# mks0601/ExAvatar_RELEASE

Hardware: NVIDIA H100
Metric: avatar train-step frames/sec (fwd+bwd raster) (higher is better)
Workload: dtype f32

## Files before the change

exavatar_release_b200/_lib.py:

```python
from __future__ import annotations

import ctypes as C
import os

_PKG = os.path.dirname(os.path.abspath(__file__))
LIB_PATH = os.path.join(_PKG, "libb200raster.so")
LIB_PATH = os.environ.get("B2R_LIB", LIB_PATH)

ABI_VERSION = 3
B2R_OK = 0
B2R_FLAG_NO_TILE_CULL = 1
B2R_FLAG_DEBUG = 2
B2R_FLAG_CTX_CLEAN = 4

_fp = C.c_void_p


class B2RScene(C.Structure):
    _fields_ = [
        ("P", C.c_int32), ("width", C.c_int32), ("height", C.c_int32), ("sh_degree", C.c_int32),
        ("sh_coeffs", C.c_int32), ("flags", C.c_uint32),
        ("scale_modifier", C.c_float), ("tanfovx", C.c_float), ("tanfovy", C.c_float),
        ("bg", _fp), ("viewmatrix", _fp), ("projmatrix", _fp), ("campos", _fp),
        ("means3D", _fp), ("shs", _fp), ("colors_precomp", _fp), ("opacities", _fp),
        ("scales", _fp), ("rotations", _fp), ("cov3D_precomp", _fp),
        ("skin_xyz", _fp), ("skin_weights", _fp), ("skin_joint_mats", _fp), ("skin_trans", _fp),
        ("skin_cam_Rinv", _fp), ("skin_cam_t", _fp), ("skin_means_out", _fp), ("skin_J", C.c_int32),
        ("sh_rows", C.c_int32),
    ]


class B2RStatus(C.Structure):
    _fields_ = [
        ("num_dups", C.c_uint64), ("dup_capacity", C.c_uint64), ("overflow", C.c_uint32), ("num_visible", C.c_uint32),
        ("consumed_fwd", C.c_uint64), ("consumed_bwd", C.c_uint64), ("token", C.c_uint64), ("reserved", C.c_uint64 * 2),
    ]


class B2RWorkspace(C.Structure):
    _fields_ = [
        ("ctx", _fp), ("ctx_bytes", C.c_size_t), ("dup_ids", _fp), ("dup_capacity", C.c_uint64),
        ("scratch", _fp), ("scratch_bytes", C.c_size_t), ("status_mirror", _fp), ("status_token", C.c_uint64),
        ("checkpoints", _fp), ("checkpoint_bytes", C.c_size_t),
    ]


class B2RView(C.Structure):
    _fields_ = [
        ("id_begin", C.c_uint32), ("id_end", C.c_uint32), ("bg", _fp), ("final_T", _fp), ("n_contrib", _fp),
        ("checkpoints", _fp), ("checkpoint_bytes", C.c_size_t), ("skip_below", C.c_uint32), ("reserved", C.c_uint32),
    ]


class B2RSkin(C.Structure):
    _fields_ = [
        ("P", C.c_int32), ("J", C.c_int32), ("V", C.c_int32), ("reserved", C.c_int32),
        ("weights", _fp), ("rows", _fp), ("joint_mats", _fp), ("trans", _fp), ("cam_Rinv", _fp), ("cam_t", _fp),
        ("xyz", _fp * 2), ("posed", _fp * 2),
    ]


class B2RMeshRender(C.Structure):
    _fields_ = [
        ("V", C.c_int32), ("F", C.c_int32), ("Vt", C.c_int32), ("C", C.c_int32),
        ("tex_height", C.c_int32), ("tex_width", C.c_int32), ("height", C.c_int32), ("width", C.c_int32),
        ("mesh", _fp), ("faces", _fp), ("vertex_uv", _fp), ("face_uv", _fp), ("texture", _fp),
        ("cam_R", _fp), ("cam_t", _fp), ("focal", _fp), ("princpt", _fp), ("keys", _fp),
        ("vf_offsets", _fp), ("vf_entries", _fp),
    ]


class B2RForwardOutputs(C.Structure):
    _fields_ = [("color", _fp), ("depth", _fp), ("alpha", _fp), ("radii", _fp)]


class B2RBackwardArgs(C.Structure):
    _fields_ = [
        ("dL_dcolor", _fp), ("dL_ddepth", _fp), ("dL_dalpha", _fp),
        ("dL_dmeans3D", _fp), ("dL_dmeans2D", _fp), ("dL_dshs", _fp), ("dL_dcolors", _fp), ("dL_dopacities", _fp),
        ("dL_dscales", _fp), ("dL_drotations", _fp), ("dL_dcov3D", _fp),
        ("flags", C.c_uint32), ("first_row", C.c_uint32),
        ("densify_grad_accum", _fp), ("densify_count", _fp), ("densify_radius_max", _fp),
        ("dL_dskin_xyz", _fp), ("dL_dskin_G", _fp),
        ("dL_dposed", _fp),
        ("densify_rows", C.c_uint32), ("reserved", C.c_uint32),
    ]


CONSUMED_FWD_DIV = 8
CONSUMED_BWD_DIV = 4

B2R_BWD_ACCUMULATE = 1
B2R_BWD_SCRATCH_ZEROED = 2


def read_status(ctx_buf) -> dict:
    s = B2RStatus.from_buffer_copy(ctx_buf[: C.sizeof(B2RStatus)].cpu().numpy().tobytes())
    return {"num_dups": int(s.num_dups), "dup_capacity": int(s.dup_capacity), "overflow": int(s.overflow),
            "num_visible": int(s.num_visible), "consumed_fwd": int(s.consumed_fwd), "consumed_bwd": int(s.consumed_bwd),
            "consumed_fwd_div": float(CONSUMED_FWD_DIV), "consumed_bwd_div": float(CONSUMED_BWD_DIV)}


SYMBOLS = [
    ("b2r_abi_version", C.c_int, []),
    ("b2r_strerror", C.c_char_p, [C.c_int]),
    ("b2r_last_cuda_error", C.c_int, []),
    ("b2r_sizeof", C.c_size_t, [C.c_int]),
    ("b2r_ctx_bytes", C.c_size_t, [C.c_int32, C.c_int32, C.c_int32]),
    ("b2r_scratch_bytes", C.c_size_t, [C.c_int32, C.c_int32, C.c_int32, C.c_uint64]),
    ("b2r_backward_scratch_bytes", C.c_size_t, [C.c_int32]),
    ("b2r_checkpoint_bytes", C.c_size_t, [C.c_int32, C.c_int32, C.c_uint64]),
    ("b2r_forward_bin", C.c_int, [C.POINTER(B2RScene), C.POINTER(B2RWorkspace), _fp]),
    ("b2r_forward_composite", C.c_int, [C.POINTER(B2RScene), C.POINTER(B2RWorkspace), C.POINTER(B2RView),
                                        C.POINTER(B2RForwardOutputs), _fp]),
    ("b2r_backward_composite", C.c_int, [C.POINTER(B2RScene), C.POINTER(B2RWorkspace), C.POINTER(B2RView),
                                         C.POINTER(B2RBackwardArgs), _fp, C.c_size_t, _fp]),
    ("b2r_backward_project", C.c_int, [C.POINTER(B2RScene), C.POINTER(B2RWorkspace), C.POINTER(B2RBackwardArgs), _fp,
                                       C.c_size_t, _fp]),
    ("b2r_forward_project", C.c_int, [C.POINTER(B2RScene), C.POINTER(B2RWorkspace), _fp, _fp]),
    ("b2r_forward_render", C.c_int, [C.POINTER(B2RScene), C.POINTER(B2RWorkspace), C.POINTER(B2RForwardOutputs), _fp]),
    ("b2r_forward", C.c_int, [C.POINTER(B2RScene), C.POINTER(B2RWorkspace), C.POINTER(B2RForwardOutputs), _fp]),
    ("b2r_backward", C.c_int, [C.POINTER(B2RScene), C.POINTER(B2RWorkspace), C.POINTER(B2RBackwardArgs), _fp,
                               C.c_size_t, _fp]),
    ("b2r_mark_visible", C.c_int, [C.c_int32, _fp, _fp, _fp, _fp]),
    ("b2r_skin_forward", C.c_int, [C.POINTER(B2RSkin), _fp]),
    ("b2r_skin_backward", C.c_int, [C.POINTER(B2RSkin), C.POINTER(_fp), C.POINTER(_fp), _fp, _fp, _fp, C.c_size_t, _fp]),
    ("b2r_skin_scratch_bytes", C.c_size_t, [C.c_int32, C.c_int32]),
    ("b2r_l1ssim_scratch_bytes", C.c_size_t, [C.c_int32, C.c_int32]),
    ("b2r_l1ssim_forward", C.c_int, [C.c_int32, C.c_int32, _fp, _fp, _fp, _fp, C.c_int32, _fp, _fp, C.c_size_t, _fp]),
    ("b2r_l1ssim_backward", C.c_int, [C.c_int32, C.c_int32, _fp, _fp, _fp, _fp, C.c_int32, _fp, _fp, _fp, C.c_size_t,
                                      _fp]),
    ("b2r_nearest_scratch_bytes", C.c_size_t, [C.c_int32, C.c_int32]),
    ("b2r_nearest_rows", C.c_int, [C.c_int32, _fp, C.c_int32, _fp, _fp, _fp, _fp, C.c_size_t, _fp]),
    ("b2r_vertex_normals", C.c_int, [C.c_int32, _fp, _fp, _fp, _fp, _fp, _fp, _fp]),
    ("b2r_mesh_render_scratch_bytes", C.c_size_t, [C.c_int32]),
    ("b2r_mesh_render_forward", C.c_int, [C.POINTER(B2RMeshRender), _fp, _fp, _fp, C.c_size_t, _fp]),
    ("b2r_mesh_render_backward", C.c_int, [C.POINTER(B2RMeshRender), _fp, _fp, _fp, _fp, C.c_size_t, _fp]),
    ("b2r_profile_enable", None, [C.c_int]),
    ("b2r_profile_read", C.c_int, [C.POINTER(C.c_double), C.POINTER(C.c_uint64), C.c_int]),
    ("b2r_launch_count", C.c_uint64, []),
    ("b2r_kernel_name", C.c_char_p, [C.c_int]),
    ("b2r_ctx_geom", _fp, [C.POINTER(B2RWorkspace), C.c_int32, C.c_int32, C.c_int32]),
    ("b2r_ctx_aux", _fp, [C.POINTER(B2RWorkspace), C.c_int32, C.c_int32, C.c_int32]),
    ("b2r_ctx_ranges", _fp, [C.POINTER(B2RWorkspace), C.c_int32, C.c_int32, C.c_int32]),
    ("b2r_ctx_final_T", _fp, [C.POINTER(B2RWorkspace), C.c_int32, C.c_int32, C.c_int32]),
    ("b2r_ctx_n_contrib", _fp, [C.POINTER(B2RWorkspace), C.c_int32, C.c_int32, C.c_int32]),
]

_lib = None


def load():
    global _lib
    if _lib is not None:
        return _lib
    if not os.path.exists(LIB_PATH):
        raise RuntimeError(
            f"b200raster: {LIB_PATH} not found. Build it with `python -m exavatar_release_b200.build_ext` "
            "(nvcc, sm_90a). There is no CPU fallback.")
    lib = C.CDLL(LIB_PATH)
    for name, restype, argtypes in SYMBOLS:
        fn = getattr(lib, name)
        fn.restype = restype
        fn.argtypes = argtypes
    if lib.b2r_abi_version() != ABI_VERSION:
        raise RuntimeError("b200raster: ABI version mismatch between the Python binding and libb200raster.so")
    for idx, cls in ((0, B2RScene), (1, B2RStatus), (2, B2RWorkspace), (3, B2RForwardOutputs), (4, B2RBackwardArgs),
                     (5, B2RView), (6, B2RSkin), (8, B2RMeshRender)):
        if lib.b2r_sizeof(idx) != C.sizeof(cls):
            raise RuntimeError(f"b200raster: struct layout drift for {cls.__name__}: "
                               f"{lib.b2r_sizeof(idx)} (C) vs {C.sizeof(cls)} (ctypes)")
    _lib = lib
    return lib


def check(rc: int, what: str):
    if rc != B2R_OK:
        lib = load()
        msg = lib.b2r_strerror(rc).decode()
        raise RuntimeError(f"b200raster: {what} failed: {msg} (code {rc}, cudaError {lib.b2r_last_cuda_error()})")
```

exavatar_release_b200/csrc/api.cu:

```cuda
#include "common.cuh"

using namespace b2r;

namespace {

int validate_scene(const B2RScene* sc) {
  if (!sc) return B2R_E_INVALID;
  if (sc->P < 0 || sc->width <= 0 || sc->height <= 0) return B2R_E_INVALID;
  if (sc->P >= (1 << 29)) return B2R_E_INVALID;
  if (sc->width > 65535 * TILE || sc->height > 32767 * TILE) return B2R_E_INVALID;
  if (!(sc->tanfovx > 0.f) || !(sc->tanfovy > 0.f)) return B2R_E_INVALID;
  if (!sc->bg || !sc->viewmatrix || !sc->projmatrix || !sc->campos) return B2R_E_INVALID;
  if (sc->sh_rows < 0 || sc->sh_rows > sc->P) return B2R_E_INVALID;
  if (sc->P > 0) {
    if (!sc->opacities) return B2R_E_INVALID;
    if (sc->skin_xyz) {
      if (!sc->skin_weights || !sc->skin_joint_mats || !sc->skin_trans) return B2R_E_INVALID;
      if (sc->skin_J <= 0 || sc->skin_J > 64) return B2R_E_INVALID;
      if (sc->skin_cam_Rinv && !sc->skin_cam_t) return B2R_E_INVALID;
    } else if (!sc->means3D) {
      return B2R_E_INVALID;
    }
    if (sc->sh_rows > 0) {
      if (!sc->shs || !sc->colors_precomp) return B2R_E_INVALID;
    } else if ((sc->shs != nullptr) == (sc->colors_precomp != nullptr)) {
      return B2R_E_INVALID;
    }
    const bool sr = sc->scales != nullptr && sc->rotations != nullptr;
    if (sr == (sc->cov3D_precomp != nullptr)) return B2R_E_INVALID;
    if ((sc->scales != nullptr) != (sc->rotations != nullptr)) return B2R_E_INVALID;
    if (sc->shs) {
      if (sc->sh_degree < 0 || sc->sh_degree > 3) return B2R_E_INVALID;
      if (sc->sh_coeffs < (sc->sh_degree + 1) * (sc->sh_degree + 1)) return B2R_E_INVALID;
      if (sc->sh_coeffs > 16) return B2R_E_INVALID;
    }
  }
  return B2R_OK;
}

int validate_ws(const B2RScene* sc, const B2RWorkspace* ws, bool need_scratch) {
  if (!ws || !ws->ctx) return B2R_E_INVALID;
  if (ws->ctx_bytes < b2r_ctx_bytes(sc->P, sc->width, sc->height)) return B2R_E_WORKSPACE;
  if (ws->dup_capacity > 0xfffffff0ull) return B2R_E_INVALID;
  if (need_scratch) {
    if (!ws->scratch) return B2R_E_INVALID;
    if (ws->scratch_bytes < b2r_scratch_bytes(sc->P, sc->width, sc->height, ws->dup_capacity)) return B2R_E_WORKSPACE;
  }
  if (ws->dup_capacity > 0 && !ws->dup_ids) return B2R_E_INVALID;
  if (ws->checkpoints && ws->checkpoint_bytes < b2r_checkpoint_bytes(sc->width, sc->height, ws->dup_capacity)) return B2R_E_WORKSPACE;
  return B2R_OK;
}

bool missing_dshs(const B2RScene* sc, const B2RBackwardArgs* a) {
  if (!sc->shs || a->dL_dshs || sc->P == 0) return false;
  return sc->sh_rows == 0 || (int64_t)a->first_row < (int64_t)sc->sh_rows;
}

int validate_skin(const B2RSkin* s) {
  if (!s) return B2R_E_INVALID;
  if (s->P < 0 || s->V <= 0) return B2R_E_INVALID;
  if (s->J <= 0 || s->J > 64) return B2R_E_INVALID;
  if (s->cam_Rinv && !s->cam_t) return B2R_E_INVALID;
  if (s->posed[1] && !s->xyz[1]) return B2R_E_INVALID;
  if (s->P > 0) {
    if (!s->weights || !s->joint_mats || !s->trans || !s->xyz[0]) return B2R_E_INVALID;
    if (!s->rows && s->V < s->P) return B2R_E_INVALID;
  }
  return B2R_OK;
}

bool valid_l1ssim_size(int32_t width, int32_t height) {
  return width > 0 && height > 0 && height <= 65535 * 16 && (int64_t)width * height <= (int64_t)1 << 31;
}

int validate_mesh_render(const B2RMeshRender* m) {
  if (!m) return B2R_E_INVALID;
  if (m->V < 0 || m->F < 0 || m->Vt < 0 || m->C < 1 || m->C > 4) return B2R_E_INVALID;
  if (m->width <= 0 || m->height <= 0 || (int64_t)m->width * m->height >= ((int64_t)1 << 31)) return B2R_E_INVALID;
  if (m->F >= (1 << 29) || m->V >= (1 << 29)) return B2R_E_INVALID;
  if (!m->cam_R || !m->cam_t || !m->focal || !m->princpt) return B2R_E_INVALID;
  if (m->F > 0) {
    if (m->V < 1 || m->Vt < 1 || m->tex_height < 1 || m->tex_width < 1) return B2R_E_INVALID;
    if ((int64_t)m->C * m->tex_height * m->tex_width >= ((int64_t)1 << 31)) return B2R_E_INVALID;
    if (!m->mesh || !m->faces || !m->vertex_uv || !m->face_uv || !m->texture) return B2R_E_INVALID;
  }
  return B2R_OK;
}

}

extern "C" {

int b2r_abi_version(void) { return B2R_ABI_VERSION; }

const char* b2r_strerror(int code) {
  switch (code) {
    case B2R_OK: return "ok";
    case B2R_E_INVALID: return "invalid argument";
    case B2R_E_WORKSPACE: return "workspace buffer too small";
    case B2R_E_CUDA: return "CUDA launch failed";
    case B2R_E_DUP_OVERFLOW: return "duplicate capacity exceeded";
    default: return "unknown error";
  }
}

int b2r_last_cuda_error(void) { return g_last_cuda_error; }

size_t b2r_sizeof(int which) {
  switch (which) {
    case 0: return sizeof(B2RScene);
    case 1: return sizeof(B2RStatus);
    case 2: return sizeof(B2RWorkspace);
    case 3: return sizeof(B2RForwardOutputs);
    case 4: return sizeof(B2RBackwardArgs);
    case 5: return sizeof(B2RView);
    case 6: return sizeof(B2RSkin);
    case 8: return sizeof(B2RMeshRender);
    default: return 0;
  }
}

size_t b2r_ctx_bytes(int32_t P, int32_t width, int32_t height) { return ctx_layout(P, width, height).total; }

size_t b2r_scratch_bytes(int32_t P, int32_t width, int32_t height, uint64_t dup_capacity) {
  return scratch_layout(P, width, height, dup_capacity).total;
}

size_t b2r_backward_scratch_bytes(int32_t P) { return align_up((size_t)(P > 0 ? P : 1) * 12 * sizeof(float)); }

size_t b2r_checkpoint_bytes(int32_t width, int32_t height, uint64_t dup_capacity) {
  const CtxLayout L = ctx_layout(0, width, height);
  const uint32_t ms = max_segments(L.tiles, dup_capacity);
  return seg_table_bytes(ms) + (size_t)ms * CK_REC_BYTES;
}

int b2r_forward_project(const B2RScene* scene, const B2RWorkspace* ws, int32_t* radii, void* stream) {
  int rc = validate_scene(scene);
  if (rc) return rc;
  rc = validate_ws(scene, ws, false);
  if (rc) return rc;
  if (scene->P > 0 && !radii) return B2R_E_INVALID;
  const Ctx cx = resolve(ws, scene->P, scene->width, scene->height);
  return launch_project(*scene, cx, radii, (cudaStream_t)stream);
}

static int forward_render(const B2RScene* scene, const B2RWorkspace* ws, const B2RForwardOutputs* out, bool rescan,
                          void* stream) {
  int rc = validate_scene(scene);
  if (rc) return rc;
  rc = validate_ws(scene, ws, true);
  if (rc) return rc;
  if (!out || !out->color || !out->depth || !out->alpha) return B2R_E_INVALID;
  const Ctx cx = resolve(ws, scene->P, scene->width, scene->height);
  rc = launch_binning(*scene, cx, rescan, (cudaStream_t)stream);
  if (rc) return rc;
  return launch_composite_fwd(*scene, cx, *out, (cudaStream_t)stream);
}

static int apply_view(Ctx& cx, const B2RScene* scene, const B2RWorkspace* ws, const B2RView* v) {
  if (!v) return B2R_OK;
  if (v->id_end < v->id_begin || (int64_t)v->id_end > (int64_t)scene->P) return B2R_E_INVALID;
  if ((v->final_T != nullptr) != (v->n_contrib != nullptr)) return B2R_E_INVALID;
  cx.id_begin = v->id_begin;
  cx.id_span = v->id_end - v->id_begin;
  cx.bg = v->bg;
  cx.skip_below = v->skip_below;
  if (v->final_T) { cx.final_T = v->final_T; cx.n_contrib = v->n_contrib; }
  if (v->checkpoints && cx.ckpt) {
    const size_t need = seg_table_bytes(cx.max_segs) + (size_t)cx.max_segs * CK_REC_BYTES;
    if (v->checkpoint_bytes < need) return B2R_E_WORKSPACE;
    cx.ckpt = (float*)((char*)v->checkpoints + seg_table_bytes(cx.max_segs));
  }
  (void)ws;
  return B2R_OK;
}

int b2r_forward_bin(const B2RScene* scene, const B2RWorkspace* ws, void* stream) {
  int rc = validate_scene(scene);
  if (rc) return rc;
  rc = validate_ws(scene, ws, true);
  if (rc) return rc;
  const Ctx cx = resolve(ws, scene->P, scene->width, scene->height);
  return launch_binning(*scene, cx, false, (cudaStream_t)stream);
}

int b2r_forward_composite(const B2RScene* scene, const B2RWorkspace* ws, const B2RView* view,
                          const B2RForwardOutputs* out, void* stream) {
  int rc = validate_scene(scene);
  if (rc) return rc;
  rc = validate_ws(scene, ws, false);
  if (rc) return rc;
  if (!out || !out->color || !out->depth || !out->alpha) return B2R_E_INVALID;
  Ctx cx = resolve(ws, scene->P, scene->width, scene->height);
  rc = apply_view(cx, scene, ws, view);
  if (rc) return rc;
  return launch_composite_fwd(*scene, cx, *out, (cudaStream_t)stream);
}

int b2r_forward_render(const B2RScene* scene, const B2RWorkspace* ws, const B2RForwardOutputs* out, void* stream) {
  return forward_render(scene, ws, out, true, stream);
}

int b2r_forward(const B2RScene* scene, const B2RWorkspace* ws, const B2RForwardOutputs* out, void* stream) {
  if (!out) return B2R_E_INVALID;
  int rc = b2r_forward_project(scene, ws, out->radii, stream);
  if (rc) return rc;
  return forward_render(scene, ws, out, false, stream);
}

int b2r_backward(const B2RScene* scene, const B2RWorkspace* ws, const B2RBackwardArgs* args, void* bwd_scratch,
                 size_t bwd_scratch_bytes, void* stream) {
  int rc = validate_scene(scene);
  if (rc) return rc;
  rc = validate_ws(scene, ws, false);
  if (rc) return rc;
  if (!args || !args->dL_dcolor || !bwd_scratch) return B2R_E_INVALID;
  if (bwd_scratch_bytes < b2r_backward_scratch_bytes(scene->P)) return B2R_E_WORKSPACE;
  if (missing_dshs(scene, args)) return B2R_E_INVALID;
  if ((int64_t)args->first_row > (int64_t)scene->P) return B2R_E_INVALID;
  if (args->dL_dposed && !scene->skin_xyz) return B2R_E_INVALID;
  const Ctx cx = resolve(ws, scene->P, scene->width, scene->height);
  float* gacc = (float*)bwd_scratch;
  rc = launch_composite_bwd(*scene, cx, *args, gacc, (cudaStream_t)stream);
  if (rc) return rc;
  return launch_project_bwd(*scene, cx, *args, gacc, (cudaStream_t)stream);
}

int b2r_backward_composite(const B2RScene* scene, const B2RWorkspace* ws, const B2RView* view, const B2RBackwardArgs* args,
                           void* bwd_scratch, size_t bwd_scratch_bytes, void* stream) {
  int rc = validate_scene(scene);
  if (rc) return rc;
  rc = validate_ws(scene, ws, false);
  if (rc) return rc;
  if (!args || !args->dL_dcolor || !bwd_scratch) return B2R_E_INVALID;
  if (bwd_scratch_bytes < b2r_backward_scratch_bytes(scene->P)) return B2R_E_WORKSPACE;
  if ((int64_t)args->first_row > (int64_t)scene->P) return B2R_E_INVALID;
  Ctx cx = resolve(ws, scene->P, scene->width, scene->height);
  rc = apply_view(cx, scene, ws, view);
  if (rc) return rc;
  return launch_composite_bwd(*scene, cx, *args, (float*)bwd_scratch, (cudaStream_t)stream);
}

int b2r_backward_project(const B2RScene* scene, const B2RWorkspace* ws, const B2RBackwardArgs* args, void* bwd_scratch,
                         size_t bwd_scratch_bytes, void* stream) {
  int rc = validate_scene(scene);
  if (rc) return rc;
  rc = validate_ws(scene, ws, false);
  if (rc) return rc;
  if (!args || !bwd_scratch) return B2R_E_INVALID;
  if (bwd_scratch_bytes < b2r_backward_scratch_bytes(scene->P)) return B2R_E_WORKSPACE;
  if (missing_dshs(scene, args)) return B2R_E_INVALID;
  if ((int64_t)args->first_row > (int64_t)scene->P) return B2R_E_INVALID;
  if (args->dL_dposed && !scene->skin_xyz) return B2R_E_INVALID;
  const Ctx cx = resolve(ws, scene->P, scene->width, scene->height);
  return launch_project_bwd(*scene, cx, *args, (const float*)bwd_scratch, (cudaStream_t)stream);
}

size_t b2r_skin_scratch_bytes(int32_t P, int32_t J) { return skin_scratch_bytes(P, J); }

int b2r_skin_forward(const B2RSkin* skin, void* stream) {
  const int rc = validate_skin(skin);
  if (rc) return rc;
  if (skin->P > 0 && !skin->posed[0]) return B2R_E_INVALID;
  return launch_skin_forward(*skin, (cudaStream_t)stream);
}

int b2r_skin_backward(const B2RSkin* skin, const float* const dL_dposed[2], float* const dL_dxyz[2], float* dL_djoint,
                      float* dL_dtrans, void* scratch, size_t scratch_bytes, void* stream) {
  const int rc = validate_skin(skin);
  if (rc) return rc;
  if (dL_dposed && dL_dposed[1] && !skin->xyz[1]) return B2R_E_INVALID;
  if ((dL_djoint || dL_dtrans) && skin->P > 0) {
    if (!scratch) return B2R_E_INVALID;
    if (scratch_bytes < skin_scratch_bytes(skin->P, skin->J)) return B2R_E_WORKSPACE;
  }
  return launch_skin_backward(*skin, dL_dposed, dL_dxyz, dL_djoint, dL_dtrans, scratch, (cudaStream_t)stream);
}

size_t b2r_l1ssim_scratch_bytes(int32_t width, int32_t height) { return l1ssim_scratch_bytes(width, height); }

int b2r_l1ssim_forward(int32_t width, int32_t height, const float* img, const float* target, const float* mask,
                       const float* bbox, int32_t with_ssim, float* out, void* scratch, size_t scratch_bytes,
                       void* stream) {
  if (!valid_l1ssim_size(width, height) || !img || !target || !out || !scratch) return B2R_E_INVALID;
  if (scratch_bytes < l1ssim_scratch_bytes(width, height)) return B2R_E_WORKSPACE;
  return launch_l1ssim_forward(width, height, img, target, mask, bbox, with_ssim != 0, out, scratch,
                               (cudaStream_t)stream);
}

int b2r_l1ssim_backward(int32_t width, int32_t height, const float* img, const float* target, const float* mask,
                        const float* bbox, int32_t with_ssim, const float* dL_dout, float* dL_dimg, const void* scratch,
                        size_t scratch_bytes, void* stream) {
  if (!valid_l1ssim_size(width, height) || !img || !target || !dL_dout || !dL_dimg) return B2R_E_INVALID;
  if (with_ssim) {
    if (!scratch) return B2R_E_INVALID;
    if (scratch_bytes < l1ssim_scratch_bytes(width, height)) return B2R_E_WORKSPACE;
  }
  return launch_l1ssim_backward(width, height, img, target, mask, bbox, with_ssim != 0, dL_dout, dL_dimg, scratch,
                                (cudaStream_t)stream);
}

size_t b2r_nearest_scratch_bytes(int32_t P, int32_t V) {
  (void)P;
  return nearest_scratch_bytes(V);
}

int b2r_nearest_rows(int32_t P, const float* queries, int32_t V, const float* targets, const uint8_t* self_map,
                     int32_t* rows, void* scratch, size_t scratch_bytes, void* stream) {
  if (P < 0 || V < 0 || V >= (1 << 29)) return B2R_E_INVALID;
  if (P == 0) return B2R_OK;
  if (V < 1 || !queries || !targets || !rows || !scratch) return B2R_E_INVALID;
  if (scratch_bytes < nearest_scratch_bytes(V)) return B2R_E_WORKSPACE;
  return launch_nearest_rows(P, queries, V, targets, self_map, rows, scratch, (cudaStream_t)stream);
}

int b2r_vertex_normals(int32_t P, const float* xyz, const int32_t* faces, const int32_t* vf_offsets,
                       const int32_t* vf_entries, const uint8_t* flip, float* normals, void* stream) {
  if (P < 0) return B2R_E_INVALID;
  if (P == 0) return B2R_OK;
  if (!xyz || !faces || !vf_offsets || !vf_entries || !normals) return B2R_E_INVALID;
  return launch_vertex_normals(P, xyz, faces, vf_offsets, vf_entries, flip, normals, (cudaStream_t)stream);
}

size_t b2r_mesh_render_scratch_bytes(int32_t F) { return mesh_render_scratch_bytes(F); }

int b2r_mesh_render_forward(const B2RMeshRender* mr, float* image, int32_t* pix_to_face, void* scratch,
                            size_t scratch_bytes, void* stream) {
  const int rc = validate_mesh_render(mr);
  if (rc) return rc;
  if (!mr->keys || !image || !pix_to_face || !scratch) return B2R_E_INVALID;
  if (scratch_bytes < mesh_render_scratch_bytes(mr->F)) return B2R_E_WORKSPACE;
  return launch_mesh_render_forward(*mr, image, pix_to_face, scratch, (cudaStream_t)stream);
}

int b2r_mesh_render_backward(const B2RMeshRender* mr, const int32_t* pix_to_face, const float* dL_dimage,
                             float* dL_dmesh, void* scratch, size_t scratch_bytes, void* stream) {
  const int rc = validate_mesh_render(mr);
  if (rc) return rc;
  if (!pix_to_face || !dL_dimage || !scratch) return B2R_E_INVALID;
  if (mr->V > 0 && (!dL_dmesh || !mr->vf_offsets || !mr->vf_entries)) return B2R_E_INVALID;
  if (scratch_bytes < mesh_render_scratch_bytes(mr->F)) return B2R_E_WORKSPACE;
  return launch_mesh_render_backward(*mr, pix_to_face, dL_dimage, dL_dmesh, scratch, (cudaStream_t)stream);
}

int b2r_mark_visible(int32_t P, const float* means3D, const float* viewmatrix, uint8_t* present, void* stream) {
  if (P < 0 || (P > 0 && (!means3D || !present)) || !viewmatrix) return B2R_E_INVALID;
  return launch_mark_visible(P, means3D, viewmatrix, present, (cudaStream_t)stream);
}

const float* b2r_ctx_geom(const B2RWorkspace* ws, int32_t P, int32_t width, int32_t height) {
  return (const float*)((const char*)ws->ctx + ctx_layout(P, width, height).geom);
}
const int32_t* b2r_ctx_aux(const B2RWorkspace* ws, int32_t P, int32_t width, int32_t height) {
  return (const int32_t*)((const char*)ws->ctx + ctx_layout(P, width, height).aux);
}
const uint32_t* b2r_ctx_ranges(const B2RWorkspace* ws, int32_t P, int32_t width, int32_t height) {
  return (const uint32_t*)((const char*)ws->ctx + ctx_layout(P, width, height).ranges);
}
const float* b2r_ctx_final_T(const B2RWorkspace* ws, int32_t P, int32_t width, int32_t height) {
  return (const float*)((const char*)ws->ctx + ctx_layout(P, width, height).final_T);
}
const uint32_t* b2r_ctx_n_contrib(const B2RWorkspace* ws, int32_t P, int32_t width, int32_t height) {
  return (const uint32_t*)((const char*)ws->ctx + ctx_layout(P, width, height).n_contrib);
}

}
```

exavatar_release_b200/csrc/binning.cu:

```cuda
#include <cstdlib>

#include "common.cuh"

namespace b2r {

__global__ void __launch_bounds__(256) scatter_kernel(const B2RScene sc, const Ctx cx) {
  const int i = blockIdx.x * blockDim.x + threadIdx.x;
  int4 aux = make_int4(0, 0, 0, 0);
  float4 g0 = make_float4(0.f, 0.f, 0.f, 0.f), g1 = g0;
  uint32_t depth_bits = 0u;
  if (i < sc.P) {
    aux = cx.aux[i];
    if (aux.z > 0) {
      const int area = ((aux.y & 0xffff) - (aux.x & 0xffff)) * ((aux.y >> 16) - (aux.x >> 16));
      depth_bits = __float_as_uint(cx.geom[i].g1.z);
      if (area > 32) {
        g0 = reinterpret_cast<const float4*>(cx.geom + i)[0];
        g1 = reinterpret_cast<const float4*>(cx.geom + i)[1];
      }
    }
  }
  const uint64_t cap = cx.dup_capacity;
  const int gx = cx.gx;
  uint32_t* cursor = cx.tile_cursor;
  uint2* keys = cx.keys;
  constexpr uint32_t NONE = 0xffffffffu;
  uint32_t pend_pos = NONE, pend_depth = 0, pend_id = 0;
  warp_replay_kept_tiles(aux.z > 0, aux.x & 0xffff, aux.x >> 16, aux.y & 0xffff, aux.y >> 16, (uint32_t)aux.w, g0.x, g0.y,
                         g0.z, g0.w, g1.x, g1.w, depth_bits, (uint32_t)i, (sc.flags & B2R_FLAG_NO_TILE_CULL) != 0, sc.width,
                         sc.height, gx, cursor, [&](uint32_t p, int, uint32_t d, uint32_t id) {
                           if (pend_pos < cap) keys[pend_pos] = make_uint2(pend_depth, pend_id);
                           pend_pos = p; pend_depth = d; pend_id = id;
                         });
  if (pend_pos < cap) keys[pend_pos] = make_uint2(pend_depth, pend_id);
}

__global__ void __launch_bounds__(256) scatter_agg_kernel(const B2RScene sc, const Ctx cx) {
  extern __shared__ uint32_t s_mem[];
  uint32_t* s_cnt = s_mem;
  uint32_t* s_base = s_mem + cx.tiles;
  for (int t = threadIdx.x; t < cx.tiles; t += blockDim.x) s_cnt[t] = 0u;
  __syncthreads();
  const int i = blockIdx.x * blockDim.x + threadIdx.x;
  int4 aux = make_int4(0, 0, 0, 0);
  float4 g0 = make_float4(0.f, 0.f, 0.f, 0.f), g1 = g0;
  uint32_t depth_bits = 0u;
  if (i < sc.P) {
    aux = cx.aux[i];
    if (aux.z > 0) {
      const int area = ((aux.y & 0xffff) - (aux.x & 0xffff)) * ((aux.y >> 16) - (aux.x >> 16));
      depth_bits = __float_as_uint(cx.geom[i].g1.z);
      if (area > 32) {
        g0 = reinterpret_cast<const float4*>(cx.geom + i)[0];
        g1 = reinterpret_cast<const float4*>(cx.geom + i)[1];
      }
    }
  }
  const int gx = cx.gx;
  const bool no_cull = (sc.flags & B2R_FLAG_NO_TILE_CULL) != 0;
  const int x0 = aux.x & 0xffff, y0 = aux.x >> 16, x1 = aux.y & 0xffff, y1 = aux.y >> 16;
  const uint32_t kept = (uint32_t)aux.w;
  warp_replay_kept_tiles(aux.z > 0, x0, y0, x1, y1, kept, g0.x, g0.y, g0.z, g0.w, g1.x, g1.w, 0u, 0u, no_cull, sc.width,
                         sc.height, gx, s_cnt, [](uint32_t, int, uint32_t, uint32_t) {});
  __syncthreads();
  for (int t = threadIdx.x; t < cx.tiles; t += blockDim.x) {
    const uint32_t c = s_cnt[t];
    if (c) {
      s_base[t] = atomicAdd(cx.tile_cursor + t, c);
      s_cnt[t] = 0u;
    }
  }
  __syncthreads();
  const uint64_t cap = cx.dup_capacity;
  uint2* keys = cx.keys;
  warp_replay_kept_tiles(aux.z > 0, x0, y0, x1, y1, kept, g0.x, g0.y, g0.z, g0.w, g1.x, g1.w, depth_bits, (uint32_t)i,
                         no_cull, sc.width, sc.height, gx, s_cnt, [&](uint32_t rank, int t, uint32_t d, uint32_t id) {
                           const uint32_t pos = s_base[t] + rank;
                           if (pos < cap) keys[pos] = make_uint2(d, id);
                         });
}


__device__ __forceinline__ unsigned match_digit(const uint32_t d, const bool valid) {
  unsigned peers = __ballot_sync(0xffffffffu, valid);
#pragma unroll
  for (int bit = 0; bit < 8; bit++) {
    const bool on = (d >> bit) & 1u;
    const unsigned b = __ballot_sync(0xffffffffu, on);
    peers &= on ? b : ~b;
  }
  return valid ? peers : 0u;
}

template <int CAP, int THREADS>
struct RadixSmem {
  static constexpr int W = THREADS / 32;
  static constexpr size_t bytes = (size_t)CAP * 12 + (size_t)W * 256 * 2 + 64;
};

template <int CAP, int THREADS, bool PAIRS = false>
__device__ __forceinline__ void radix_sort_tile(const uint2* src, uint32_t* dst, const int n, unsigned char* smem_raw,
                                                uint32_t* maxid) {
  constexpr int W = THREADS / 32;
  constexpr int ROWS = CAP / (W * 32);
  static_assert(CAP % (W * 32) == 0, "a warp's share must be whole rows");
  uint32_t* keyA = reinterpret_cast<uint32_t*>(smem_raw);
  uint32_t* keyB = keyA + CAP;
  uint16_t* idxA = reinterpret_cast<uint16_t*>(keyB + CAP);
  uint16_t* idxB = idxA + CAP;
  uint16_t* hist = idxB + CAP;
  uint32_t* misc = reinterpret_cast<uint32_t*>(hist + W * 256);
  const int tid = threadIdx.x, lane = tid & 31, warp = tid >> 5;

  if (tid == 0) { misc[0] = 0u; misc[1] = 0xffffffffu; }
  __syncthreads();
  uint32_t vor = 0u, vand = 0xffffffffu;
  for (int i = tid; i < n; i += THREADS) {
    const uint32_t k = src[i].x;
    keyA[i] = k;
    idxA[i] = (uint16_t)i;
    vor |= k;
    vand &= k;
  }
  vor = __reduce_or_sync(0xffffffffu, vor);
  vand = __reduce_and_sync(0xffffffffu, vand);
  if (lane == 0) { atomicOr(&misc[0], vor); atomicAnd(&misc[1], vand); }
  __syncthreads();
  const uint32_t differ = misc[0] ^ misc[1];

  const int chunk = (((n + W - 1) / W) + 31) & ~31;
  const int c_begin = min(warp * chunk, n), c_end = min(c_begin + chunk, n);
  uint32_t* kin = keyA; uint32_t* kout = keyB;
  uint16_t* iin = idxA; uint16_t* iout = idxB;
  for (int pass = 0; pass < 4; pass++) {
    const int shift = 8 * pass;
    if (((differ >> shift) & 0xffu) == 0u) continue;
    for (int i = tid; i < W * 256; i += THREADS) hist[i] = 0;
    __syncthreads();
    uint16_t* myhist = hist + warp * 256;
    unsigned row_peers[ROWS];
#pragma unroll
    for (int r = 0; r < ROWS; r++) {
      const int base = c_begin + 32 * r;
      row_peers[r] = 0u;
      if (base < c_end) {
        const int i = base + lane;
        const bool valid = i < c_end;
        const uint32_t d = valid ? ((kin[i] >> shift) & 0xffu) : (256u + lane);
        const unsigned peers = match_digit(d, valid);
        row_peers[r] = peers;
        if (valid && (peers & ((1u << lane) - 1u)) == 0u) myhist[d] = (uint16_t)(myhist[d] + __popc(peers));
        __syncwarp();
      }
    }
    __syncthreads();
    constexpr int DPT = THREADS >= 256 ? 1 : 256 / THREADS;
    constexpr int SCAN_THREADS = 256 / DPT;
    uint32_t tot[DPT];
    uint32_t total = 0;
    if (tid < SCAN_THREADS) {
#pragma unroll
      for (int r = 0; r < DPT; r++) {
        const int d = tid * DPT + r;
        uint32_t run = 0;
        for (int w = 0; w < W; w++) {
          const uint32_t t = hist[w * 256 + d];
          hist[w * 256 + d] = (uint16_t)run;
          run += t;
        }
        tot[r] = run;
        total += run;
      }
    }
    uint32_t incl = total;
#pragma unroll
    for (int o = 1; o < 32; o <<= 1) {
      const uint32_t v = __shfl_up_sync(0xffffffffu, incl, o);
      if (lane >= o) incl += v;
    }
    if (tid < SCAN_THREADS && lane == 31) misc[2 + warp] = incl;
    __syncthreads();
    if (tid < SCAN_THREADS) {
      uint32_t base = incl - total;
      for (int w = 0; w < warp; w++) base += misc[2 + w];
#pragma unroll
      for (int r = 0; r < DPT; r++) {
        const int d = tid * DPT + r;
        for (int w = 0; w < W; w++) hist[w * 256 + d] = (uint16_t)(hist[w * 256 + d] + base);
        base += tot[r];
      }
    }
    __syncthreads();
#pragma unroll
    for (int r = 0; r < ROWS; r++) {
      const int base = c_begin + 32 * r;
      if (base < c_end) {
        const int i = base + lane;
        const bool valid = i < c_end;
        const uint32_t k = valid ? kin[i] : 0u;
        const uint32_t d = (k >> shift) & 0xffu;
        const unsigned peers = row_peers[r];
        const unsigned below = peers & ((1u << lane) - 1u);
        uint32_t start = 0;
        if (valid && below == 0u) {
          start = myhist[d];
          myhist[d] = (uint16_t)(start + __popc(peers));
        }
        start = __shfl_sync(0xffffffffu, start, valid ? __ffs(peers) - 1 : lane);
        if (valid) {
          const uint32_t o = start + __popc(below);
          kout[o] = k;
          iout[o] = iin[i];
        }
        __syncwarp();
      }
    }
    __syncthreads();
    { uint32_t* t = kin; kin = kout; kout = t; }
    { uint16_t* t = iin; iin = iout; iout = t; }
  }
  uint32_t* ids = kout;
  uint32_t vmax = 0u;
  for (int i = tid; i < n; i += THREADS) {
    const uint32_t id = src[iin[i]].y;
    ids[i] = id;
    vmax = max(vmax, id);
  }
  vmax = __reduce_max_sync(0xffffffffu, vmax);
  if (lane == 0 && vmax) atomicMax(maxid, vmax);
  __syncthreads();
  for (;;) {
    int changed = 0;
#pragma unroll
    for (int phase = 0; phase < 2; phase++) {
      for (int i = 2 * tid + phase; i + 1 < n; i += 2 * THREADS) {
        if (kin[i] == kin[i + 1]) {
          const uint32_t a = ids[i], b = ids[i + 1];
          if (a > b) { ids[i] = b; ids[i + 1] = a; changed = 1; }
        }
      }
      __syncthreads();
    }
    if (!__syncthreads_or(changed)) break;
  }
  if (PAIRS) {
    uint2* out = const_cast<uint2*>(src);
    for (int i = tid; i < n; i += THREADS) out[i] = make_uint2(kin[i], ids[i]);
  } else {
    for (int i = tid; i < n; i += THREADS) dst[i] = ids[i];
  }
  __syncthreads();
}

constexpr int WSORT_CAP = 1 << SORT_CTA_SHIFT;
constexpr size_t WSORT_BYTES = (size_t)WSORT_CAP * 12 + 256 * 2;

__device__ __forceinline__ void warp_sort_tile(const uint2* __restrict__ src, uint32_t* __restrict__ dst, const int n,
                                               unsigned char* smem_warp, uint32_t* __restrict__ maxid) {
  const int lane = threadIdx.x & 31;
  const unsigned below_mask = (1u << lane) - 1u;
  if (n <= 0) return;
  if (n <= 32) {
    const uint2 kv = lane < n ? src[lane] : make_uint2(0xffffffffu, 0xffffffffu);
    const uint32_t m = __reduce_max_sync(0xffffffffu, lane < n ? kv.y : 0u);
    if (lane == 0) *maxid = m;
    const unsigned long long me = ((unsigned long long)kv.x << 32) | kv.y;
    int rank = 0;
    for (int j = 0; j < n; j++) {
      const unsigned long long o = __shfl_sync(0xffffffffu, me, j);
      rank += (o < me) ? 1 : 0;
    }
    if (lane < n) dst[rank] = kv.y;
    return;
  }
  uint32_t* keyA = reinterpret_cast<uint32_t*>(smem_warp);
  uint32_t* keyB = keyA + WSORT_CAP;
  uint16_t* idxA = reinterpret_cast<uint16_t*>(keyB + WSORT_CAP);
  uint16_t* idxB = idxA + WSORT_CAP;
  uint16_t* hist = idxB + WSORT_CAP;
  uint32_t vor = 0u, vand = 0xffffffffu;
  for (int i = lane; i < n; i += 32) {
    const uint32_t k = src[i].x;
    keyA[i] = k;
    idxA[i] = (uint16_t)i;
    vor |= k;
    vand &= k;
  }
  const uint32_t differ = __reduce_or_sync(0xffffffffu, vor) ^ __reduce_and_sync(0xffffffffu, vand);
  __syncwarp();
  uint32_t* kin = keyA; uint32_t* kout = keyB;
  uint16_t* iin = idxA; uint16_t* iout = idxB;
  for (int pass = 0; pass < 4; pass++) {
    const int shift = 8 * pass;
    if (((differ >> shift) & 0xffu) == 0u) continue;
    reinterpret_cast<uint4*>(hist)[lane] = make_uint4(0u, 0u, 0u, 0u);
    __syncwarp();
    constexpr int CACHED = 8;
    unsigned row_peers[CACHED];
#pragma unroll
    for (int r = 0; r < CACHED; r++) {
      const int base = 32 * r;
      row_peers[r] = 0u;
      if (base < n) {
        const int i = base + lane;
        const bool valid = i < n;
        const uint32_t d = valid ? ((kin[i] >> shift) & 0xffu) : (256u + lane);
        const unsigned peers = match_digit(d, valid);
        row_peers[r] = peers;
        if (valid && (peers & below_mask) == 0u) hist[d] = (uint16_t)(hist[d] + __popc(peers));
        __syncwarp();
      }
    }
    for (int base = 32 * CACHED; base < n; base += 32) {
      const int i = base + lane;
      const bool valid = i < n;
      const uint32_t d = valid ? ((kin[i] >> shift) & 0xffu) : (256u + lane);
      const unsigned peers = match_digit(d, valid);
      if (valid && (peers & below_mask) == 0u) hist[d] = (uint16_t)(hist[d] + __popc(peers));
      __syncwarp();
    }
    uint32_t c[8], total = 0;
#pragma unroll
    for (int r = 0; r < 8; r++) { c[r] = hist[8 * lane + r]; total += c[r]; }
    uint32_t incl = total;
#pragma unroll
    for (int o = 1; o < 32; o <<= 1) {
      const uint32_t v = __shfl_up_sync(0xffffffffu, incl, o);
      if (lane >= o) incl += v;
    }
    uint32_t run = incl - total;
#pragma unroll
    for (int r = 0; r < 8; r++) { hist[8 * lane + r] = (uint16_t)run; run += c[r]; }
    __syncwarp();
    auto place_row = [&](const int base, const bool cached, const unsigned cached_peers) {
        const int i = base + lane;
        const bool valid = i < n;
        const uint32_t k = valid ? kin[i] : 0u;
        const uint32_t d = valid ? ((k >> shift) & 0xffu) : (256u + lane);
        const unsigned peers = cached ? cached_peers : match_digit(d, valid);
        const unsigned below = peers & below_mask;
        uint32_t start = 0;
        if (valid && below == 0u) {
          start = hist[d];
          hist[d] = (uint16_t)(start + __popc(peers));
        }
        start = __shfl_sync(0xffffffffu, start, valid ? __ffs(peers) - 1 : lane);
        if (valid) {
          const uint32_t o = start + __popc(below);
          kout[o] = k;
          iout[o] = iin[i];
        }
        __syncwarp();
    };
#pragma unroll
    for (int r = 0; r < CACHED; r++)
      if (32 * r < n) place_row(32 * r, true, row_peers[r]);
    for (int base = 32 * CACHED; base < n; base += 32) place_row(base, false, 0u);
    { uint32_t* t = kin; kin = kout; kout = t; }
    { uint16_t* t = iin; iin = iout; iout = t; }
  }
  uint32_t* ids = kout;
  uint32_t vmax = 0u;
  for (int i = lane; i < n; i += 32) {
    const uint32_t id = src[iin[i]].y;
    ids[i] = id;
    vmax = max(vmax, id);
  }
  vmax = __reduce_max_sync(0xffffffffu, vmax);
  if (lane == 0) *maxid = vmax;
  __syncwarp();
  for (;;) {
    bool changed = false;
#pragma unroll
    for (int phase = 0; phase < 2; phase++) {
      for (int i = 2 * lane + phase; i + 1 < n; i += 64) {
        if (kin[i] == kin[i + 1]) {
          const uint32_t a = ids[i], b = ids[i + 1];
          if (a > b) { ids[i] = b; ids[i + 1] = a; changed = true; }
        }
      }
      __syncwarp();
    }
    if (!__any_sync(0xffffffffu, changed)) break;
  }
  for (int i = lane; i < n; i += 32) dst[i] = ids[i];
  __syncwarp();
}

template <int CAP, int THREADS>
__global__ void __launch_bounds__(THREADS) sort_mixed_kernel(const Ctx cx) {
  extern __shared__ __align__(16) unsigned char smem_raw[];
  B2R_TRACE_BEGIN();
  const unsigned long long cls = cx.status->reserved[0];
  const int n_large = (int)(cls & 0xffffffffull), n_ge512 = (int)(cls >> 32);
  const int n_chunks = (int)cx.status->reserved[1];
  const int n_cta = n_ge512 - n_large;
  const int n_warp_items = (cx.tiles - n_ge512 + (THREADS / 32) - 1) / (THREADS / 32);
  const int items = n_chunks + n_cta + n_warp_items;
  int last_n = 0;
  for (int b = blockIdx.x; b < items; b += gridDim.x) {
    if (b < n_chunks) {
      int lo = 0, hi = n_large - 1;
      while (lo < hi) {
        const int mid = (lo + hi + 1) >> 1;
        if ((int)cx.chunk_start[mid] <= b) lo = mid; else hi = mid - 1;
      }
      const uint32_t tile = cx.tile_order[lo];
      const uint2 r = cx.ranges[tile];
      const int off = (b - (int)cx.chunk_start[lo]) * SORT_CHUNK;
      const int len = min(SORT_CHUNK, (int)(r.y - r.x) - off);
      if (len > 1) radix_sort_tile<CAP, THREADS, true>(cx.keys + r.x + off, nullptr, len, smem_raw, cx.tile_maxid + tile);
      else if (len == 1 && threadIdx.x == 0) atomicMax(cx.tile_maxid + tile, cx.keys[r.x + off].y);
      last_n = len;
    } else if (b < n_chunks + n_cta) {
      const uint32_t tile = cx.tile_order[n_large + (b - n_chunks)];
      const uint2 r = cx.ranges[tile];
      const int n = (int)(r.y - r.x);
      const uint2* src = cx.keys + r.x;
      uint32_t* dst = cx.dup_ids + r.x;
      if (n > 32) {
        radix_sort_tile<CAP, THREADS>(src, dst, n, smem_raw, cx.tile_maxid + tile);
      } else {
        if (threadIdx.x < 32) warp_sort_tile(src, dst, n, smem_raw, cx.tile_maxid + tile);
        __syncthreads();
      }
      last_n = n;
    } else {
      const int warp = threadIdx.x >> 5;
      const int t = n_ge512 + (b - n_chunks - n_cta) * (THREADS / 32) + warp;
      if (t < cx.tiles) {
        const uint32_t tile = cx.tile_order[t];
        const uint2 r = cx.ranges[tile];
        last_n = -(int)(r.y - r.x);
        warp_sort_tile(cx.keys + r.x, cx.dup_ids + r.x, (int)(r.y - r.x), smem_raw + (size_t)warp * WSORT_BYTES,
                       cx.tile_maxid + tile);
      }
    }
  }
  B2R_TRACE_END(last_n);
}

constexpr int MERGE_TABLE = 1024;
__global__ void __launch_bounds__(256) merge_chunks_kernel(const Ctx cx) {
  const int n_large = (int)(cx.status->reserved[0] & 0xffffffffull);
  const int n_chunks = (int)cx.status->reserved[1];
  if ((int)blockIdx.x >= n_chunks) return;
  __shared__ uint2 other[SORT_CHUNK];
  __shared__ uint32_t table[MERGE_TABLE];
  const int tid = threadIdx.x;
  const int n_tab = min(n_large, MERGE_TABLE);
  for (int i = tid; i < n_tab; i += 256) table[i] = cx.chunk_start[i];
  __syncthreads();
  constexpr int PER = SORT_CHUNK / 256;
  for (int b = blockIdx.x; b < n_chunks; b += gridDim.x) {
    int lo = 0, hi = n_large - 1;
    while (lo < hi) {
      const int mid = (lo + hi + 1) >> 1;
      const int cs = mid < n_tab ? (int)table[mid] : (int)cx.chunk_start[mid];
      if (cs <= b) lo = mid; else hi = mid - 1;
    }
    const uint2 r = cx.ranges[cx.tile_order[lo]];
    const int n = (int)(r.y - r.x);
    const int c = b - (int)(lo < n_tab ? table[lo] : cx.chunk_start[lo]);
    const uint2* pairs = cx.keys + r.x;
    const int chunks = (n + SORT_CHUNK - 1) / SORT_CHUNK;
    const int len = min(SORT_CHUNK, n - c * SORT_CHUNK);
    unsigned long long key[PER];
    uint32_t id[PER];
    int rank[PER];
#pragma unroll
    for (int j = 0; j < PER; j++) {
      const int i = j * 256 + tid;
      const uint2 me = i < len ? pairs[c * SORT_CHUNK + i] : make_uint2(0u, 0u);
      key[j] = ((unsigned long long)me.x << 32) | me.y;
      id[j] = me.y;
      rank[j] = i;
    }
    for (int c2 = 0; c2 < chunks; c2++) {
      if (c2 == c) continue;
      const uint2* q = pairs + c2 * SORT_CHUNK;
      const int len2 = min(SORT_CHUNK, n - c2 * SORT_CHUNK);
      __syncthreads();
#pragma unroll
      for (int j = 0; j < PER; j++) {
        const int i = j * 256 + tid;
        if (i < len2) other[i] = q[i];
      }
      __syncthreads();
      int l[PER];
#pragma unroll
      for (int j = 0; j < PER; j++) l[j] = 0;
#pragma unroll
      for (int step = SORT_CHUNK / 2; step >= 1; step >>= 1) {
#pragma unroll
        for (int j = 0; j < PER; j++) {
          const int probe = l[j] + step;
          if (probe <= len2) {
            const uint2 v = other[probe - 1];
            if ((((unsigned long long)v.x << 32) | v.y) < key[j]) l[j] = probe;
          }
        }
      }
      if (len2 == SORT_CHUNK) {
#pragma unroll
        for (int j = 0; j < PER; j++) {
          if (l[j] == SORT_CHUNK - 1) {
            const uint2 v = other[SORT_CHUNK - 1];
            if ((((unsigned long long)v.x << 32) | v.y) < key[j]) l[j] = SORT_CHUNK;
          }
        }
      }
#pragma unroll
      for (int j = 0; j < PER; j++) rank[j] += l[j];
    }
#pragma unroll
    for (int j = 0; j < PER; j++)
      if (j * 256 + tid < len) cx.dup_ids[r.x + rank[j]] = id[j];
  }
}

constexpr int SORT_SMALL = SORT_CHUNK;

int launch_binning(const B2RScene& sc, const Ctx& cx, bool rescan, cudaStream_t st) {
  if (rescan) {
    Ctx quiet = cx;
    quiet.status_mirror = nullptr;
    launch_tile_scan(quiet, st);
  }
  if (sc.P > 0) {
    ProfScope p(K_SCATTER, st);
    const size_t smem = (size_t)cx.tiles * 8;
    if (cx.tiles <= 2048) {
      cudaFuncSetAttribute(scatter_agg_kernel, cudaFuncAttributeMaxDynamicSharedMemorySize, 96 * 1024);
      launch_k(scatter_agg_kernel, (sc.P + 255) / 256, 256, smem, st, true, sc, cx);
    } else {
      launch_k(scatter_kernel, (sc.P + 255) / 256, 256, 0, st, true, sc, cx);
    }
  }
  const int sms = device_sm_count();
  constexpr int ST = 256;
  constexpr size_t cta_bytes = RadixSmem<SORT_SMALL, ST>::bytes, warp_bytes = (ST / 32) * WSORT_BYTES;
  constexpr size_t small_bytes = cta_bytes > warp_bytes ? cta_bytes : warp_bytes;
  cudaFuncSetAttribute(sort_mixed_kernel<SORT_SMALL, ST>, cudaFuncAttributeMaxDynamicSharedMemorySize, (int)small_bytes);
  {
    ProfScope p(K_SORT_SMALL, st);
    launch_k(sort_mixed_kernel<SORT_SMALL, ST>, cx.tiles, ST, small_bytes, st, true, cx);
  }
  {
    ProfScope p(K_SORT_LARGE, st);
    launch_k(merge_chunks_kernel, 2 * sms, 256, 0, st, true, cx);
  }
  return check_launch();
}

}

#ifdef B2R_CTA_TRACE
extern "C" int b2r_debug_trace_sort(unsigned long long* buf) {
  return (int)cudaMemcpyToSymbol(b2r::g_cta_trace, &buf, sizeof(buf));
}
#endif
```

exavatar_release_b200/csrc/common.cuh:

```cuda
#pragma once
#include <cuda_runtime.h>
#include <stdint.h>

#include "../../include/b200raster.h"

namespace b2r {

constexpr int TILE = 16;
constexpr int TILE_PIX = TILE * TILE;
constexpr float K_NEAR = 0.2f;
constexpr float K_DILATE = 0.3f;
constexpr float K_ALPHA_MAX = 0.99f;
constexpr float K_ALPHA_MIN = 1.0f / 255.0f;
constexpr float K_T_MIN = 0.0001f;
constexpr float K_FRUSTUM = 1.3f;
constexpr float K_EPS_W = 0.0000001f;
constexpr float K_EIG_FLOOR = 0.1f;
constexpr float LOG2E = 1.4426950408889634f;
constexpr float INV_LOG2E = 0.6931471805599453f;
constexpr float CULL_MARGIN2 = 0.02f;

#ifndef SORT_CTA_SHIFT
#define SORT_CTA_SHIFT 9
#endif
constexpr int SORT_CHUNK = 2048;
#ifndef SEG_SHIFT
#define SEG_SHIFT 9
#endif
constexpr int SEG = 1 << SEG_SHIFT;
constexpr int CK_PLANE0 = TILE_PIX * 4;
constexpr int CK_REC_FLOATS = TILE_PIX * 4 + TILE_PIX * 2;
constexpr size_t CK_REC_BYTES = (size_t)CK_REC_FLOATS * 4;
enum { CLS_N_LARGE = 0,
       CLS_N_GE512 = 1,
       CLS_N_MULTI = 2,
       CLS_N_CHUNKS = 3,
       CLS_TOTAL_SEGS = 4,
       CLS_N_GE1024 = 5,
       CLS_VIS_ACC = 6,
       CLS_SCAN_FINAL = 7,
       CLS_COUNT = 8 };
constexpr size_t ALIGN = 256;
__host__ __device__ inline size_t align_up(size_t v) { return (v + ALIGN - 1) / ALIGN * ALIGN; }

struct Geom {
  float4 g0;
  float4 g1;
  float4 g2;
};
static_assert(sizeof(Geom) == 48, "Geom must be 48 bytes");

struct CtxLayout {
  size_t status, geom, aux, ranges, tile_count, tile_cursor, tile_order, chunk_start, seg_start, classes, tile_maxid,
      final_T, n_contrib, total;
  int gx, gy, tiles;
};
__host__ __device__ inline CtxLayout ctx_layout(int P, int W, int H) {
  CtxLayout L;
  L.gx = (W + TILE - 1) / TILE;
  L.gy = (H + TILE - 1) / TILE;
  L.tiles = L.gx * L.gy;
  size_t Pn = P > 0 ? (size_t)P : 1, N = (size_t)W * H;
  size_t o = 0;
  L.status = o; o += align_up(sizeof(B2RStatus));
  L.geom = o; o += align_up(Pn * sizeof(Geom));
  L.aux = o; o += align_up(Pn * 16);
  L.ranges = o; o += align_up((size_t)L.tiles * 8);
  L.tile_count = o; o += align_up((size_t)L.tiles * 4);
  L.tile_cursor = o; o += align_up((size_t)L.tiles * 4);
  L.tile_order = o; o += align_up((size_t)L.tiles * 4);
  L.chunk_start = o; o += align_up((size_t)L.tiles * 4);
  L.seg_start = o; o += align_up((size_t)L.tiles * 4);
  L.classes = o; o += align_up((size_t)CLS_COUNT * 4);
  L.tile_maxid = o; o += align_up((size_t)L.tiles * 4);
  L.final_T = o; o += align_up(N * 4);
  L.n_contrib = o; o += align_up(N * 4);
  L.total = o;
  return L;
}

struct ScratchLayout {
  size_t keys, total;
};
__host__ __device__ inline ScratchLayout scratch_layout(int P, int W, int H, uint64_t cap) {
  (void)P; (void)W; (void)H;
  ScratchLayout S;
  size_t o = 0;
  S.keys = o; o += align_up((size_t)(cap > 0 ? cap : 1) * 8);
  S.total = o;
  return S;
}

struct Ctx {
  B2RStatus* status;
  Geom* geom;
  int4* aux;
  uint2* ranges;
  float* final_T;
  uint32_t* n_contrib;
  uint32_t* dup_ids;
  uint64_t dup_capacity;
  uint32_t* tile_count;
  uint32_t* tile_cursor;
  uint32_t* tile_order;
  uint32_t* chunk_start;
  uint2* keys;
  uint64_t* status_mirror;
  uint64_t status_token;
  int gx, gy, tiles;
  uint32_t* seg_start;
  uint32_t* classes;
  uint2* seg_table;
  float* ckpt;
  uint32_t max_segs;
  uint32_t id_begin, id_span;
  const float* bg;
  uint32_t* tile_maxid;
  uint32_t skip_below;
};

__host__ __device__ inline uint32_t max_segments(int tiles, uint64_t cap) { return (uint32_t)(cap / SEG) + (uint32_t)tiles; }
__host__ __device__ inline size_t seg_table_bytes(uint32_t max_segs) { return align_up((size_t)max_segs * 8); }

inline Ctx resolve(const B2RWorkspace* ws, int P, int W, int H) {
  CtxLayout L = ctx_layout(P, W, H);
  ScratchLayout S = scratch_layout(P, W, H, ws->dup_capacity);
  char* c = (char*)ws->ctx;
  char* s = (char*)ws->scratch;
  Ctx x;
  x.status = (B2RStatus*)(c + L.status);
  x.geom = (Geom*)(c + L.geom);
  x.aux = (int4*)(c + L.aux);
  x.ranges = (uint2*)(c + L.ranges);
  x.final_T = (float*)(c + L.final_T);
  x.n_contrib = (uint32_t*)(c + L.n_contrib);
  x.dup_ids = ws->dup_ids;
  x.dup_capacity = ws->dup_capacity;
  x.tile_count = (uint32_t*)(c + L.tile_count);
  x.tile_cursor = (uint32_t*)(c + L.tile_cursor);
  x.tile_order = (uint32_t*)(c + L.tile_order);
  x.chunk_start = (uint32_t*)(c + L.chunk_start);
  x.keys = s ? (uint2*)(s + S.keys) : nullptr;
  x.status_mirror = ws->status_mirror;
  x.status_token = ws->status_token;
  x.gx = L.gx; x.gy = L.gy; x.tiles = L.tiles;
  x.seg_start = (uint32_t*)(c + L.seg_start);
  x.classes = (uint32_t*)(c + L.classes);
  x.seg_table = nullptr; x.ckpt = nullptr; x.max_segs = 0;
  if (ws->checkpoints) {
    const uint32_t ms = max_segments(L.tiles, ws->dup_capacity);
    if (ws->checkpoint_bytes >= seg_table_bytes(ms) + (size_t)ms * CK_REC_BYTES) {
      x.seg_table = (uint2*)ws->checkpoints;
      x.ckpt = (float*)((char*)ws->checkpoints + seg_table_bytes(ms));
      x.max_segs = ms;
    }
  }
  x.id_begin = 0; x.id_span = 0xffffffffu;
  x.bg = nullptr;
  x.tile_maxid = (uint32_t*)(c + L.tile_maxid);
  x.skip_below = 0;
  return x;
}

__device__ __forceinline__ float region_max_p2(float sx, float sy, float A2, float B2, float C2, float x0, float y0,
                                               float x1, float y1) {
  const float lx = sx - x1, hx = sx - x0;
  const float ly = sy - y1, hy = sy - y0;
  const bool in_x = (lx <= 0.f) && (hx >= 0.f);
  const bool in_y = (ly <= 0.f) && (hy >= 0.f);
  if (in_x && in_y) return 0.f;
  float best = -INFINITY;
  if (!in_x) {
    const float ex = lx > 0.f ? lx : hx;
    float dy = __fdividef(-B2 * ex, 2.f * C2);
    dy = fminf(fmaxf(dy, ly), hy);
    best = fmaxf(best, A2 * ex * ex + B2 * ex * dy + C2 * dy * dy);
  }
  if (!in_y) {
    const float ey = ly > 0.f ? ly : hy;
    float dx = __fdividef(-B2 * ey, 2.f * A2);
    dx = fminf(fmaxf(dx, lx), hx);
    best = fmaxf(best, A2 * dx * dx + B2 * dx * ey + C2 * ey * ey);
  }
  return best;
}

struct RowCull {
  float sx, sy, A2, B2, nD4, fA4t, dy_ext, dys, inv2A;
  int mode;
};
__device__ __forceinline__ RowCull row_cull_setup(float sx, float sy, float A2, float B2, float C2, float thr2, bool no_cull) {
  RowCull rc;
  rc.sx = sx; rc.sy = sy; rc.A2 = A2; rc.B2 = B2;
  rc.mode = (no_cull || thr2 == -INFINITY) ? 1 : 0;
  const float D = B2 * B2 - 4.f * A2 * C2;
  const float k = __fdividef(4.f * thr2, -D);
  rc.dy_ext = sqrtf(A2 * k);
  const float dx_top = sqrtf(C2 * k);
  rc.dys = __fdividef(-B2, 2.f * C2) * dx_top;
  rc.nD4 = D;
  rc.fA4t = 4.f * A2 * thr2;
  rc.inv2A = __fdividef(1.f, 2.f * A2);
  if (rc.mode == 0 && !(rc.dy_ext >= 0.f)) rc.mode = 2;
  return rc;
}
constexpr float ROW_PAD = 0.01f;
__device__ __forceinline__ void row_kept_columns(const RowCull& rc, int ty, int x0, int x1, int W, int H, int& tlo, int& thi) {
  tlo = x0; thi = x1 - 1;
  if (rc.mode == 1) return;
  if (rc.mode == 2) { thi = tlo - 1; return; }
  const float y0 = (float)(ty * TILE), y1 = fminf(y0 + (float)(TILE - 1), (float)(H - 1));
  const float lo = fmaxf(rc.sy - y1, -rc.dy_ext), hi = fminf(rc.sy - y0, rc.dy_ext);
  if (!(lo <= hi)) { thi = tlo - 1; return; }
  const float dyr = fminf(fmaxf(rc.dys, lo), hi), dyl = fminf(fmaxf(-rc.dys, lo), hi);
  const float disc_r = fmaxf(rc.nD4 * dyr * dyr + rc.fA4t, 0.f), disc_l = fmaxf(rc.nD4 * dyl * dyl + rc.fA4t, 0.f);
  const float dx_hi = (-rc.B2 * dyr - sqrtf(disc_r)) * rc.inv2A;
  const float dx_lo = (-rc.B2 * dyl + sqrtf(disc_l)) * rc.inv2A;
  const float xl = rc.sx - dx_hi - ROW_PAD, xr = rc.sx - dx_lo + ROW_PAD;
  if (!(xl <= (float)(W - 1))) { thi = tlo - 1; return; }
  tlo = max(x0, (int)ceilf((xl - (float)(TILE - 1)) * (1.f / TILE)));
  thi = min(x1 - 1, (int)floorf(xr * (1.f / TILE)));
}

__device__ __forceinline__ int rect_row(int t, float inv_w) { return (int)(((float)t + 0.5f) * inv_w); }

constexpr int KEPT_SMALL = 4;
#ifndef WALK_ROW_COST_N
#define WALK_ROW_COST_N 40
#endif
constexpr unsigned WALK_ROW_COST = WALK_ROW_COST_N, WALK_TILE_COST = 10u, WALK_BCAST_COST = 30u;

__device__ __forceinline__ uint32_t bit_run(int pos, int cnt) { return (cnt >= 32 ? 0xffffffffu : ((1u << cnt) - 1u)) << pos; }

__device__ __forceinline__ uint32_t warp_count_kept_tiles(bool active, int x0, int y0, int x1, int y1, float px, float py,
                                                          float A2, float B2, float C2, float thr2, bool no_cull, int W,
                                                          int H, int gx, uint32_t* table) {
  const int lane = threadIdx.x & 31;
  const int w = x1 - x0, h = y1 - y0;
  const int area = active ? w * h : 0;
  uint32_t kept = 0u;
  const bool big = area > KEPT_SMALL;
  const unsigned own_cost = area ? (unsigned)h * WALK_ROW_COST + (unsigned)area * WALK_TILE_COST : 0u;
  const unsigned coop_cost = big ? WALK_BCAST_COST + (unsigned)((h + 31) >> 5) * (WALK_ROW_COST + (unsigned)w * WALK_TILE_COST) : 0u;
  const unsigned max_own = __reduce_max_sync(0xffffffffu, own_cost);
  const unsigned sum_coop = __reduce_add_sync(0xffffffffu, coop_cost);
  const bool all_private = max_own <= sum_coop + 64u;
  if (area > 0 && (all_private || !big)) {
    const RowCull rc = row_cull_setup(px, py, A2, B2, C2, thr2, no_cull);
    for (int ty = y0; ty < y1; ty++) {
      int tlo, thi;
      row_kept_columns(rc, ty, x0, x1, W, H, tlo, thi);
      if (tlo <= thi) {
        if (area <= 32) kept |= bit_run((ty - y0) * w + (tlo - x0), thi - tlo + 1);
        uint32_t* row = table + ty * gx;
        for (int tx = tlo; tx <= thi; tx++) atomicAdd(row + tx, 1u);
      }
    }
  }
  unsigned mask = all_private ? 0u : __ballot_sync(0xffffffffu, big);
  while (mask) {
    const int src = __ffs(mask) - 1;
    mask &= mask - 1;
    const int bx0 = __shfl_sync(0xffffffffu, x0, src), by0 = __shfl_sync(0xffffffffu, y0, src);
    const int bx1 = __shfl_sync(0xffffffffu, x1, src), by1 = __shfl_sync(0xffffffffu, y1, src);
    const float spx = __shfl_sync(0xffffffffu, px, src), spy = __shfl_sync(0xffffffffu, py, src);
    const float sA = __shfl_sync(0xffffffffu, A2, src), sB = __shfl_sync(0xffffffffu, B2, src);
    const float sC = __shfl_sync(0xffffffffu, C2, src), sT = __shfl_sync(0xffffffffu, thr2, src);
    const RowCull rc = row_cull_setup(spx, spy, sA, sB, sC, sT, no_cull);
    const int bw = bx1 - bx0;
    const bool small = bw * (by1 - by0) <= 32;
    uint32_t bits = 0u;
    for (int ty = by0 + lane; ty < by1; ty += 32) {
      int tlo, thi;
      row_kept_columns(rc, ty, bx0, bx1, W, H, tlo, thi);
      if (tlo <= thi) {
        if (small) bits |= bit_run((ty - by0) * bw + (tlo - bx0), thi - tlo + 1);
        uint32_t* row = table + ty * gx;
        for (int tx = tlo; tx <= thi; tx++) atomicAdd(row + tx, 1u);
      }
    }
    bits = __reduce_or_sync(0xffffffffu, bits);
    if (lane == src) kept = bits;
  }
  return kept;
}

template <typename F>
__device__ __forceinline__ void warp_replay_kept_tiles(bool active, int x0, int y0, int x1, int y1, uint32_t kept, float px,
                                                       float py, float A2, float B2, float C2, float thr2, uint32_t u0,
                                                       uint32_t u1, bool no_cull, int W, int H, int gx, uint32_t* table,
                                                       F&& post) {
  const int lane = threadIdx.x & 31;
  const int w = x1 - x0, h = y1 - y0;
  const int area = active ? w * h : 0;
  if (area > 0 && area <= 32) {
    const float inv_w = __frcp_rn((float)w);
    const int tile0 = y0 * gx + x0;
    for (uint32_t m = kept; m; m &= m - 1u) {
      const int t = __ffs(m) - 1;
      const int r = rect_row(t, inv_w);
      const int tile = tile0 + r * gx + (t - r * w);
      post(atomicAdd(table + tile, 1u), tile, u0, u1);
    }
  }
  const bool big = area > 32;
  const unsigned own_cost = big ? (unsigned)h * WALK_ROW_COST + (unsigned)area * WALK_TILE_COST : 0u;
  const unsigned coop_cost = big ? WALK_BCAST_COST + (unsigned)((h + 31) >> 5) * (WALK_ROW_COST + (unsigned)w * WALK_TILE_COST) : 0u;
  const unsigned sum_coop = __reduce_add_sync(0xffffffffu, coop_cost);
  if (sum_coop == 0u) return;
  const unsigned max_own = __reduce_max_sync(0xffffffffu, own_cost);
  if (max_own <= sum_coop) {
    if (big) {
      const RowCull rc = row_cull_setup(px, py, A2, B2, C2, thr2, no_cull);
      for (int ty = y0; ty < y1; ty++) {
        int tlo, thi;
        row_kept_columns(rc, ty, x0, x1, W, H, tlo, thi);
        for (int tx = tlo; tx <= thi; tx++) {
          const int tile = ty * gx + tx;
          post(atomicAdd(table + tile, 1u), tile, u0, u1);
        }
      }
    }
    return;
  }
  unsigned mask = __ballot_sync(0xffffffffu, big);
  while (mask) {
    const int src = __ffs(mask) - 1;
    mask &= mask - 1;
    const int bx0 = __shfl_sync(0xffffffffu, x0, src), by0 = __shfl_sync(0xffffffffu, y0, src);
    const int bx1 = __shfl_sync(0xffffffffu, x1, src), by1 = __shfl_sync(0xffffffffu, y1, src);
    const uint32_t s0 = __shfl_sync(0xffffffffu, u0, src), s1 = __shfl_sync(0xffffffffu, u1, src);
    const float spx = __shfl_sync(0xffffffffu, px, src), spy = __shfl_sync(0xffffffffu, py, src);
    const float sA = __shfl_sync(0xffffffffu, A2, src), sB = __shfl_sync(0xffffffffu, B2, src);
    const float sC = __shfl_sync(0xffffffffu, C2, src), sT = __shfl_sync(0xffffffffu, thr2, src);
    const RowCull rc = row_cull_setup(spx, spy, sA, sB, sC, sT, no_cull);
    for (int ty = by0 + lane; ty < by1; ty += 32) {
      int tlo, thi;
      row_kept_columns(rc, ty, bx0, bx1, W, H, tlo, thi);
      for (int tx = tlo; tx <= thi; tx++) {
        const int tile = ty * gx + tx;
        post(atomicAdd(table + tile, 1u), tile, s0, s1);
      }
    }
  }
}

__device__ __forceinline__ float ex2_approx(float x) {
  float y;
  asm("ex2.approx.ftz.f32 %0, %1;" : "=f"(y) : "f"(x));
  return y;
}

__device__ __forceinline__ void cp_async16(void* smem_dst, const void* gmem_src) {
  unsigned s = (unsigned)__cvta_generic_to_shared(smem_dst);
  asm volatile("cp.async.cg.shared.global [%0], [%1], 16;\n" ::"r"(s), "l"(gmem_src));
}
__device__ __forceinline__ void cp_async_commit() { asm volatile("cp.async.commit_group;\n" ::); }
template <int N>
__device__ __forceinline__ void cp_async_wait() { asm volatile("cp.async.wait_group %0;\n" ::"n"(N)); }

__device__ __forceinline__ void red_add_v4(float* addr, float a, float b, float c, float d) {
  asm volatile("red.global.add.v4.f32 [%0], {%1, %2, %3, %4};\n" ::"l"(addr), "f"(a), "f"(b), "f"(c), "f"(d) : "memory");
}

template <int MODE>
__device__ __forceinline__ void stage_rows(float* __restrict__ wstage, float* __restrict__ gptr, const int L, const int nrows,
                                           const unsigned row_mask) {
  const int lane = threadIdx.x & 31;
  const int S = L | 1;
  if (L == 48 && (reinterpret_cast<uintptr_t>(gptr) & 15) == 0) {
    float4* g4 = reinterpret_cast<float4*>(gptr);
    const int n4 = nrows * 12;
    float4 v[12];
    if (MODE != 1) {
#pragma unroll
      for (int u = 0; u < 12; u++) {
        const int j = lane + 32 * u;
        const bool rd = j < n4 && (MODE == 0 || ((row_mask >> (j / 12)) & 1u));
        v[u] = rd ? (MODE == 0 ? __ldg(g4 + j) : g4[j]) : make_float4(0.f, 0.f, 0.f, 0.f);
      }
    }
#pragma unroll
    for (int u = 0; u < 12; u++) {
      const int j = lane + 32 * u;
      const int r = j / 12, c = (j - r * 12) * 4;
      float* w = wstage + r * S + c;
      if (j < n4) {
        if (MODE == 0) {
          w[0] = v[u].x; w[1] = v[u].y; w[2] = v[u].z; w[3] = v[u].w;
        } else if ((row_mask >> r) & 1u) {
          if (MODE == 1) g4[j] = make_float4(w[0], w[1], w[2], w[3]);
          else g4[j] = make_float4(v[u].x + w[0], v[u].y + w[1], v[u].z + w[2], v[u].w + w[3]);
        }
      }
    }
    return;
  }
  const int total = nrows * L;
  for (int e0 = lane; e0 < total; e0 += 32 * 8) {
    float v[8];
    if (MODE != 1) {
#pragma unroll
      for (int u = 0; u < 8; u++) {
        const int e = e0 + 32 * u;
        v[u] = (e < total && (MODE == 0 || ((row_mask >> (e / L)) & 1u))) ? gptr[e] : 0.f;
      }
    }
#pragma unroll
    for (int u = 0; u < 8; u++) {
      const int e = e0 + 32 * u;
      if (e < total) {
        const int r = e / L, c = e - r * L;
        float* w = wstage + r * S + c;
        if (MODE == 0) *w = v[u];
        else if ((row_mask >> r) & 1u) gptr[e] = MODE == 1 ? *w : v[u] + *w;
      }
    }
  }
}

int launch_project(const B2RScene& sc, const Ctx& cx, int32_t* radii, cudaStream_t st);
int launch_binning(const B2RScene& sc, const Ctx& cx, bool rescan, cudaStream_t st);
void launch_tile_scan(const Ctx& cx, cudaStream_t st);
int launch_composite_fwd(const B2RScene& sc, const Ctx& cx, const B2RForwardOutputs& out, cudaStream_t st);
int launch_composite_bwd(const B2RScene& sc, const Ctx& cx, const B2RBackwardArgs& a, float* gacc, cudaStream_t st);

int launch_project_bwd(const B2RScene& sc, const Ctx& cx, const B2RBackwardArgs& a, const float* gacc, cudaStream_t st);
int launch_mark_visible(int P, const float* means3D, const float* view, uint8_t* present, cudaStream_t st);
int launch_skin_forward(const B2RSkin& s, cudaStream_t st);
int launch_skin_backward(const B2RSkin& s, const float* const dposed[2], float* const dxyz[2], float* djoint,
                         float* dtrans, void* scratch, cudaStream_t st);
size_t skin_scratch_bytes(int P, int J);
int launch_l1ssim_forward(int W, int H, const float* img, const float* target, const float* mask, const float* bbox,
                          bool with_ssim, float* out, void* scratch, cudaStream_t st);
int launch_l1ssim_backward(int W, int H, const float* img, const float* target, const float* mask, const float* bbox,
                           bool with_ssim, const float* dout, float* dimg, const void* scratch, cudaStream_t st);
size_t l1ssim_scratch_bytes(int W, int H);
int launch_nearest_rows(int P, const float* queries, int V, const float* targets, const uint8_t* self_map,
                        int32_t* rows, void* scratch, cudaStream_t st);
size_t nearest_scratch_bytes(int V);
int launch_vertex_normals(int P, const float* xyz, const int32_t* faces, const int32_t* vf_offsets,
                          const int32_t* vf_entries, const uint8_t* flip, float* normals, cudaStream_t st);
size_t mesh_render_scratch_bytes(int F);
int launch_mesh_render_forward(const B2RMeshRender& m, float* image, int32_t* pix_to_face, void* scratch,
                               cudaStream_t st);
int launch_mesh_render_backward(const B2RMeshRender& m, const int32_t* pix_to_face, const float* dimage, float* dmesh,
                                void* scratch, cudaStream_t st);

enum KernelId { K_PROJECT = 0, K_TILE_SCAN, K_SCATTER, K_SORT_SMALL, K_SORT_LARGE, K_COMPOSITE_FWD, K_COMPOSITE_BWD,
                K_PROJECT_BWD, K_MISC };
struct ProfScope {
  int id;
  cudaStream_t st;
  bool on;
  cudaEvent_t a;
  ProfScope(int id, cudaStream_t st, int launches = 1);
  ~ProfScope();
};

#ifdef B2R_CTA_TRACE
static __device__ unsigned long long* g_cta_trace;
__device__ __forceinline__ unsigned long long trace_now() {
  unsigned long long t;
  asm volatile("mov.u64 %0, %globaltimer;" : "=l"(t));
  return t;
}
__device__ __forceinline__ void trace_end(unsigned long long t0, int n) {
  if (threadIdx.x == 0 && g_cta_trace) {
    unsigned smid;
    asm volatile("mov.u32 %0, %smid;" : "=r"(smid));
    unsigned long long* d = g_cta_trace + 4ull * blockIdx.x;
    d[0] = t0; d[1] = trace_now(); d[2] = smid; d[3] = (unsigned long long)n;
  }
}
#define B2R_TRACE_BEGIN() const unsigned long long trace_t0 = trace_now()
#define B2R_TRACE_END(n) trace_end(trace_t0, (n))
#else
#define B2R_TRACE_BEGIN()
#define B2R_TRACE_END(n)
#endif

int launch_priority(bool high);
int device_sm_count();
template <typename... KArgs, typename... Args>
inline void launch_k(void (*kernel)(KArgs...), dim3 grid, dim3 block, size_t smem, cudaStream_t st, bool high,
                     Args... args) {
  cudaLaunchConfig_t cfg = {};
  cfg.gridDim = grid;
  cfg.blockDim = block;
  cfg.dynamicSmemBytes = smem;
  cfg.stream = st;
  cudaLaunchAttribute attr[1];
  attr[0].id = cudaLaunchAttributePriority;
  attr[0].val.priority = launch_priority(high);
  cfg.attrs = attr;
  cfg.numAttrs = 1;
  cudaLaunchKernelEx(&cfg, kernel, static_cast<KArgs>(args)...);
}

extern int g_last_cuda_error;
inline int check_launch() {
  cudaError_t e = cudaGetLastError();
  if (e != cudaSuccess) {
    g_last_cuda_error = (int)e;
    return B2R_E_CUDA;
  }
  return B2R_OK;
}

}
```

exavatar_release_b200/csrc/project.cu:

```cuda
#include "gaussian_math.cuh"

namespace b2r {

int g_last_cuda_error = 0;

__device__ __forceinline__ void sh_to_rgb(int deg, const float* __restrict__ sh, const float3 mean, const Cam& cam,
                                          float* rgb, uint32_t& clamp_bits) {
  float dx = mean.x - cam.campos[0], dy = mean.y - cam.campos[1], dz = mean.z - cam.campos[2];
  const float n = sqrtf(dx * dx + dy * dy + dz * dz);
  const float x = dx / n, y = dy / n, z = dz / n;
  clamp_bits = 0;
#pragma unroll
  for (int c = 0; c < 3; c++) {
    auto SH = [&](int k) { return sh[k * 3 + c]; };
    float r = B2R_SH_C0 * SH(0);
    if (deg > 0) {
      r = r - B2R_SH_C1 * y * SH(1) + B2R_SH_C1 * z * SH(2) - B2R_SH_C1 * x * SH(3);
      if (deg > 1) {
        const float xx = x * x, yy = y * y, zz = z * z, xy = x * y, yz = y * z, xz = x * z;
        r = r + c_SH_C2[0] * xy * SH(4) + c_SH_C2[1] * yz * SH(5) + c_SH_C2[2] * (2.f * zz - xx - yy) * SH(6) +
            c_SH_C2[3] * xz * SH(7) + c_SH_C2[4] * (xx - yy) * SH(8);
        if (deg > 2) {
          r = r + c_SH_C3[0] * y * (3.f * xx - yy) * SH(9) + c_SH_C3[1] * xy * z * SH(10) +
              c_SH_C3[2] * y * (4.f * zz - xx - yy) * SH(11) + c_SH_C3[3] * z * (2.f * zz - 3.f * xx - 3.f * yy) * SH(12) +
              c_SH_C3[4] * x * (4.f * zz - xx - yy) * SH(13) + c_SH_C3[5] * z * (xx - yy) * SH(14) +
              c_SH_C3[6] * x * (xx - 3.f * yy) * SH(15);
        }
      }
    }
    r += 0.5f;
    if (r < 0.f) clamp_bits |= 1u << c;
    rgb[c] = fmaxf(r, 0.f);
  }
}

#ifndef PROJ_MIN_BLOCKS
#define PROJ_MIN_BLOCKS 4
#endif
template <bool MIXED>
__global__ void __launch_bounds__(256, PROJ_MIN_BLOCKS) project_kernel(const B2RScene sc, const Ctx cx, int32_t* __restrict__ radii,
                                                      const int aggregate) {
  extern __shared__ uint32_t s_cnt[];
  if (aggregate) {
    for (int t = threadIdx.x; t < cx.tiles; t += blockDim.x) s_cnt[t] = 0u;
    __syncthreads();
  }
  const int i = blockIdx.x * blockDim.x + threadIdx.x;
  const float* shrow = nullptr;
  if (sc.shs) {
    const int lane = threadIdx.x & 31, warp = threadIdx.x >> 5;
    const int L = sc.sh_coeffs * 3, S = L | 1;
    float* wstage = reinterpret_cast<float*>(s_cnt + (aggregate ? cx.tiles : 0)) + (size_t)warp * 32 * S;
    const int row0 = blockIdx.x * blockDim.x + warp * 32;
    const int nrows = min(32, (MIXED ? sc.sh_rows : sc.P) - row0);
    if (nrows > 0) stage_rows<0>(wstage, const_cast<float*>(sc.shs) + (size_t)row0 * L, L, nrows, 0xffffffffu);
    __syncwarp();
    shrow = wstage + lane * S;
  }
  const float* wrow = nullptr;
  if (sc.skin_xyz) {
    const int lane = threadIdx.x & 31, warp = threadIdx.x >> 5;
    const int J = sc.skin_J, S = J | 1;
    float* base = reinterpret_cast<float*>(s_cnt + (aggregate ? cx.tiles : 0));
    if (sc.shs) base += (size_t)8 * 32 * ((sc.sh_coeffs * 3) | 1);
    float* wstage = base + (size_t)warp * 32 * S;
    const int row0 = blockIdx.x * blockDim.x + warp * 32;
    const int nrows = min(32, sc.P - row0);
    if (nrows > 0) stage_rows<0>(wstage, const_cast<float*>(sc.skin_weights) + (size_t)row0 * J, J, nrows, 0xffffffffu);
    __syncwarp();
    wrow = wstage + lane * S;
  }
  const Cam cam = load_cam(sc);
  bool visible = false;
  Geom g;
  g.g0 = make_float4(0.f, 0.f, 0.f, 0.f);
  g.g1 = make_float4(0.f, 0.f, 0.f, INFINITY);
  g.g2 = make_float4(0.f, 0.f, 0.f, 0.f);
  int4 aux = make_int4(0, 0, 0, 0);
  if (i < sc.P) {
    float3 p;
    if (wrow) {
      p = skin_position(sc, i, wrow).world;
      if (sc.skin_means_out) {
        sc.skin_means_out[3 * (size_t)i] = p.x;
        sc.skin_means_out[3 * (size_t)i + 1] = p.y;
        sc.skin_means_out[3 * (size_t)i + 2] = p.z;
      }
    } else {
      p = make_float3(__ldg(sc.means3D + 3 * (size_t)i), __ldg(sc.means3D + 3 * (size_t)i + 1),
                      __ldg(sc.means3D + 3 * (size_t)i + 2));
    }
    const float3 pv = xform4x3(p, cam.v);
    if (pv.z > K_NEAR) {
      const float ph_x = dot4_rn(cam.p[0], p.x, cam.p[4], p.y, cam.p[8], p.z, cam.p[12]);
      const float ph_y = dot4_rn(cam.p[1], p.x, cam.p[5], p.y, cam.p[9], p.z, cam.p[13]);
      const float ph_w = dot4_rn(cam.p[3], p.x, cam.p[7], p.y, cam.p[11], p.z, cam.p[15]);
      const float pw = __fdiv_rn(1.f, __fadd_rn(ph_w, K_EPS_W));
      float c6[6];
      if (sc.cov3D_precomp) {
#pragma unroll
        for (int k = 0; k < 6; k++) c6[k] = __ldg(sc.cov3D_precomp + 6 * (size_t)i + k);
      } else {
        const float3 s = make_float3(__ldg(sc.scales + 3 * (size_t)i), __ldg(sc.scales + 3 * (size_t)i + 1),
                                     __ldg(sc.scales + 3 * (size_t)i + 2));
        const float* qp = sc.rotations + 4 * (size_t)i;
        const float4 q = make_float4(__ldg(qp), __ldg(qp + 1), __ldg(qp + 2), __ldg(qp + 3));
        cov3d_from_scale_rot(s, sc.scale_modifier, q, c6);
      }
      Ewa e;
      ewa_project(pv, c6, cam, e);
      const float det = e.a * e.c - e.b * e.b;
      if (det != 0.f) {
        const float det_inv = 1.f / det;
        const float conx = e.c * det_inv, cony = -e.b * det_inv, conz = e.a * det_inv;
        const float mid = 0.5f * (e.a + e.c);
        const float root = sqrtf(fmaxf(K_EIG_FLOOR, mid * mid - det));
        const float lam = fmaxf(mid + root, mid - root);
        const int radius = (int)ceilf(3.f * sqrtf(lam));
        const float px = __fmul_rn(__fadd_rn(__fmul_rn(__fadd_rn(__fmul_rn(ph_x, pw), 1.f), (float)cam.W), -1.f), 0.5f);
        const float py = __fmul_rn(__fadd_rn(__fmul_rn(__fadd_rn(__fmul_rn(ph_y, pw), 1.f), (float)cam.H), -1.f), 0.5f);
        int x0 = (int)((px - (float)radius) / (float)TILE), y0 = (int)((py - (float)radius) / (float)TILE);
        int x1 = (int)((px + (float)radius + (float)(TILE - 1)) / (float)TILE);
        int y1 = (int)((py + (float)radius + (float)(TILE - 1)) / (float)TILE);
        x0 = min(cx.gx, max(0, x0)); y0 = min(cx.gy, max(0, y0));
        x1 = min(cx.gx, max(0, x1)); y1 = min(cx.gy, max(0, y1));
        if ((x1 - x0) * (y1 - y0) != 0) {
          visible = true;
          const float o = __ldg(sc.opacities + i);
          float rgb[3];
          uint32_t bits = 0;
          if (sc.shs && (!MIXED || i < sc.sh_rows)) {
            sh_to_rgb(sc.sh_degree, shrow, p, cam, rgb, bits);
          } else {
            rgb[0] = __ldg(sc.colors_precomp + 3 * (size_t)i);
            rgb[1] = __ldg(sc.colors_precomp + 3 * (size_t)i + 1);
            rgb[2] = __ldg(sc.colors_precomp + 3 * (size_t)i + 2);
          }
          const float A2 = -0.5f * LOG2E * conx, B2 = -LOG2E * cony, C2 = -0.5f * LOG2E * conz;
          float thr2;
          const bool concave = (A2 < 0.f) && (C2 < 0.f) && (4.f * A2 * C2 > B2 * B2) && (det > 0.f);
          if (!(o > 0.f)) thr2 = INFINITY;
          else if (!concave) thr2 = -INFINITY;
          else thr2 = -log2f(255.f * o) - CULL_MARGIN2;
          g.g0 = make_float4(px, py, A2, B2);
          g.g1 = make_float4(C2, o, pv.z, thr2);
          g.g2 = make_float4(rgb[0], rgb[1], rgb[2], __uint_as_float((bits << 29) | (uint32_t)i));
          aux = make_int4(x0 | (y0 << 16), x1 | (y1 << 16), radius, 0);
        }
      }
    }
    radii[i] = aux.z;
    float4* gp = reinterpret_cast<float4*>(cx.geom + i);
    gp[0] = g.g0;
    gp[1] = g.g1;
    gp[2] = g.g2;
  }
  {
    const int gx = cx.gx;
    uint32_t* tile_count = aggregate ? s_cnt : cx.tile_count;
    aux.w = (int)warp_count_kept_tiles(visible, aux.x & 0xffff, aux.x >> 16, aux.y & 0xffff, aux.y >> 16, g.g0.x, g.g0.y,
                                       g.g0.z, g.g0.w, g.g1.x, g.g1.w, (sc.flags & B2R_FLAG_NO_TILE_CULL) != 0, sc.width,
                                       sc.height, gx, tile_count);
    if (i < sc.P) cx.aux[i] = aux;
  }
  if (blockIdx.x == 0 && threadIdx.x == 0) cx.classes[CLS_SCAN_FINAL] = 0u;
  const unsigned vis = __ballot_sync(0xffffffffu, visible);
  if ((threadIdx.x & 31) == 0 && vis) atomicAdd(&cx.classes[CLS_VIS_ACC], (uint32_t)__popc(vis));
  if (aggregate) {
    __syncthreads();
    for (int t = threadIdx.x; t < cx.tiles; t += blockDim.x) {
      const uint32_t c = s_cnt[t];
      if (c) atomicAdd(cx.tile_count + t, c);
    }
  }
}

__global__ void __launch_bounds__(1024) tile_scan_kernel(const Ctx cx, const int final) {
  if (final == 2 && cx.classes[CLS_SCAN_FINAL] != 0u) return;
  __shared__ uint64_t warp_sums[32];
  __shared__ uint64_t carry_s;
  const int lane = threadIdx.x & 31, warp = threadIdx.x >> 5;
  if (threadIdx.x == 0) carry_s = 0;
  __syncthreads();
  for (int base = 0; base < cx.tiles; base += 1024) {
    const int t = base + threadIdx.x;
    const uint64_t v = t < cx.tiles ? cx.tile_count[t] : 0;
    uint64_t inc = v;
#pragma unroll
    for (int d = 1; d < 32; d <<= 1) {
      const uint64_t n = __shfl_up_sync(0xffffffffu, inc, d);
      if (lane >= d) inc += n;
    }
    if (lane == 31) warp_sums[warp] = inc;
    __syncthreads();
    if (warp == 0) {
      uint64_t w = warp_sums[lane];
#pragma unroll
      for (int d = 1; d < 32; d <<= 1) {
        const uint64_t n = __shfl_up_sync(0xffffffffu, w, d);
        if (lane >= d) w += n;
      }
      warp_sums[lane] = w;
    }
    __syncthreads();
    const uint64_t carry = carry_s;
    const uint64_t excl = carry + (warp > 0 ? warp_sums[warp - 1] : 0) + inc - v;
    if (t < cx.tiles) {
      const uint64_t cap = cx.dup_capacity;
      const uint32_t s = (uint32_t)(excl < cap ? excl : cap);
      const uint32_t e = (uint32_t)(excl + v < cap ? excl + v : cap);
      cx.ranges[t] = make_uint2(s, e);
      cx.tile_cursor[t] = s;
    }
    __syncthreads();
    if (threadIdx.x == 1023) carry_s = carry + warp_sums[31];
    __syncthreads();
  }
  __shared__ uint32_t bin_cursor[34];
  __shared__ uint32_t n_large_s, n_multi_s;
  if (threadIdx.x < 34) bin_cursor[threadIdx.x] = 0;
  __syncthreads();
  auto bin_of = [](uint32_t n) { return n == 0 ? 33 : __clz(n); };
  for (int t = threadIdx.x; t < cx.tiles; t += blockDim.x) atomicAdd(&bin_cursor[bin_of(cx.tile_count[t])], 1u);
  __syncthreads();
  if (threadIdx.x == 0) {
    uint32_t run = 0;
    for (int b = 0; b < 34; b++) {
      const uint32_t c = bin_cursor[b];
      bin_cursor[b] = run;
      run += c;
    }
    cx.status->reserved[0] = (unsigned long long)bin_cursor[21] | ((unsigned long long)bin_cursor[32 - SORT_CTA_SHIFT] << 32);
    n_large_s = bin_cursor[21];
    n_multi_s = cx.ckpt ? bin_cursor[32 - SEG_SHIFT] : 0u;
    cx.classes[CLS_N_LARGE] = bin_cursor[21];
    cx.classes[CLS_N_GE512] = bin_cursor[23];
    cx.classes[CLS_N_GE1024] = bin_cursor[22];
    cx.classes[CLS_N_MULTI] = n_multi_s;
  }
  __syncthreads();
  for (int t = threadIdx.x; t < cx.tiles; t += blockDim.x) {
    const uint32_t pos = atomicAdd(&bin_cursor[bin_of(cx.tile_count[t])], 1u);
    cx.tile_order[pos] = (uint32_t)t;
  }
  __syncthreads();
  __shared__ uint32_t wsum[32];
  auto scan_units = [&](const uint32_t n_tiles, const int shift, uint32_t* out) -> uint32_t {
    uint32_t run = 0;
    for (uint32_t base = 0; base < n_tiles; base += 1024) {
      const uint32_t t = base + threadIdx.x;
      uint32_t c = 0;
      if (t < n_tiles) {
        const uint2 r = cx.ranges[cx.tile_order[t]];
        c = (r.y - r.x + (1u << shift) - 1u) >> shift;
      }
      uint32_t incl = c;
#pragma unroll
      for (int d = 1; d < 32; d <<= 1) {
        const uint32_t v = __shfl_up_sync(0xffffffffu, incl, d);
        if (lane >= d) incl += v;
      }
      if (lane == 31) wsum[warp] = incl;
      __syncthreads();
      if (warp == 0) {
        uint32_t w = wsum[lane];
#pragma unroll
        for (int d = 1; d < 32; d <<= 1) {
          const uint32_t v = __shfl_up_sync(0xffffffffu, w, d);
          if (lane >= d) w += v;
        }
        wsum[lane] = w;
      }
      __syncthreads();
      if (t < n_tiles) out[t] = run + (warp > 0 ? wsum[warp - 1] : 0u) + incl - c;
      run += wsum[31];
      __syncthreads();
    }
    return run;
  };
  static_assert(SORT_CHUNK == 2048 && SEG == (1 << SEG_SHIFT), "scan_units takes the unit as a shift");
  const uint32_t n_chunks = scan_units(n_large_s, 11, cx.chunk_start);
  uint32_t segs = scan_units(n_multi_s, SEG_SHIFT, cx.seg_start);
  __syncthreads();
  if (threadIdx.x == 0) {
    cx.status->reserved[1] = n_chunks;
    cx.classes[CLS_N_CHUNKS] = n_chunks;
    if (segs > cx.max_segs) { segs = 0; cx.classes[CLS_N_MULTI] = 0; n_multi_s = 0; }
    cx.classes[CLS_TOTAL_SEGS] = segs;
  }
  __syncthreads();
  for (uint32_t t = threadIdx.x; t < n_multi_s; t += blockDim.x) {
    const uint2 r = cx.ranges[cx.tile_order[t]];
    const uint32_t c = (r.y - r.x + SEG - 1) / SEG, s0 = cx.seg_start[t];
    for (uint32_t k = 0; k < c; k++) cx.seg_table[s0 + k] = make_uint2(t, k);
  }
  if (final) {
    for (int t = threadIdx.x; t < cx.tiles; t += blockDim.x) {
      cx.tile_count[t] = 0u;
      cx.tile_maxid[t] = 0u;
    }
  }
  if (threadIdx.x == 0) {
    const uint64_t total = carry_s;
    cx.status->num_visible = cx.classes[CLS_VIS_ACC];
    if (final) {
      cx.classes[CLS_VIS_ACC] = 0u;
      cx.classes[CLS_SCAN_FINAL] = 1u;
    }
    cx.status->consumed_fwd = 0;
    cx.status->consumed_bwd = 0;
    cx.status->num_dups = total;
    cx.status->dup_capacity = cx.dup_capacity;
    cx.status->overflow = total > cx.dup_capacity ? 1u : 0u;
    cx.status->token = cx.status_token;
    if (cx.status_mirror) {
      volatile uint64_t* m = cx.status_mirror;
      m[0] = total;
      __threadfence_system();
      m[1] = cx.status_token;
    }
  }
}

__global__ void status_reset_kernel(const Ctx cx) {
  const int t = blockIdx.x * blockDim.x + threadIdx.x;
  if (t < cx.tiles) {
    cx.tile_count[t] = 0u;
    cx.tile_maxid[t] = 0u;
  }
  if (t == 0) {
    B2RStatus* s = cx.status;
    s->num_dups = 0;
    s->overflow = 0;
    s->num_visible = 0;
    s->consumed_fwd = 0;
    s->consumed_bwd = 0;
    cx.classes[CLS_VIS_ACC] = 0u;
    cx.classes[CLS_SCAN_FINAL] = 0u;
  }
}

__global__ void mark_visible_kernel(int P, const float* __restrict__ means3D, const float* __restrict__ view,
                                    uint8_t* __restrict__ present) {
  const int i = blockIdx.x * blockDim.x + threadIdx.x;
  if (i >= P) return;
  const float x = means3D[3 * (size_t)i], y = means3D[3 * (size_t)i + 1], z = means3D[3 * (size_t)i + 2];
  const float vz = dot4_rn(view[2], x, view[6], y, view[10], z, view[14]);
  present[i] = vz > K_NEAR ? 1 : 0;
}

int launch_project(const B2RScene& sc, const Ctx& cx, int32_t* radii, cudaStream_t st) {
  const bool clean = (sc.flags & B2R_FLAG_CTX_CLEAN) != 0;
  if (!clean) { ProfScope p(K_MISC, st); launch_k(status_reset_kernel, (cx.tiles + 1023) / 1024, 1024, 0, st, true, cx); }
  if (sc.P > 0) {
    ProfScope p(K_PROJECT, st);
    const int aggregate = cx.tiles <= 2048;
    const size_t smem = (aggregate ? (size_t)cx.tiles * 4 : 0) +
                        (sc.shs ? (size_t)8 * 32 * ((sc.sh_coeffs * 3) | 1) * sizeof(float) : 0) +
                        (sc.skin_xyz ? (size_t)8 * 32 * (sc.skin_J | 1) * sizeof(float) : 0);
    auto kern = sc.sh_rows > 0 ? project_kernel<true> : project_kernel<false>;
    cudaFuncSetAttribute(kern, cudaFuncAttributeMaxDynamicSharedMemorySize, 160 * 1024);
    launch_k(kern, (sc.P + 255) / 256, 256, smem, st, true, sc, cx, radii, aggregate);
  }
  { ProfScope p(K_TILE_SCAN, st); launch_k(tile_scan_kernel, 1, 1024, 0, st, true, cx, cx.dup_capacity > 0 ? 1 : 0); }
  return check_launch();
}

void launch_tile_scan(const Ctx& cx, cudaStream_t st) {
  ProfScope p(K_TILE_SCAN, st);
  launch_k(tile_scan_kernel, 1, 1024, 0, st, true, cx, 2);
}

int launch_mark_visible(int P, const float* means3D, const float* view, uint8_t* present, cudaStream_t st) {
  ProfScope p(K_MISC, st, P > 0 ? 1 : 0);
  if (P > 0) launch_k(mark_visible_kernel, (P + 255) / 256, 256, 0, st, true, P, means3D, view, present);
  return check_launch();
}

}
```

exavatar_release_b200/csrc/project_bwd.cu:

```cuda
#include "gaussian_math.cuh"

namespace b2r {

template <bool MIXED>
__device__ __forceinline__ void project_bwd_one(const B2RScene& sc, const Ctx& cx, const B2RBackwardArgs& out,
                                                const float* __restrict__ gacc, const int i, const size_t oi,
                                                const bool visible, const int4 aux, float* shrow,
                                                const float* wrow) {
  const int M = sc.sh_coeffs;
  const bool accumulate = (out.flags & B2R_BWD_ACCUMULATE) != 0;

  float dm[3] = {0.f, 0.f, 0.f}, dm2[2] = {0.f, 0.f}, dcol[3] = {0.f, 0.f, 0.f}, dop = 0.f;
  float dS[6] = {0.f, 0.f, 0.f, 0.f, 0.f, 0.f};
  float dscale[3] = {0.f, 0.f, 0.f}, dq[4] = {0.f, 0.f, 0.f, 0.f};
  uint32_t clamp_bits = 0;
  float3 p = make_float3(0.f, 0.f, 0.f);
  Cam cam;
  Skin skin;
  const bool posed_in = wrow != nullptr && out.dL_dposed != nullptr;
  if (posed_in && !visible) skin = skin_position(sc, i, wrow);

  if (visible) {
    cam = load_cam(sc);
    const float4 q0 = reinterpret_cast<const float4*>(gacc)[3 * (size_t)i];
    const float4 q1 = reinterpret_cast<const float4*>(gacc)[3 * (size_t)i + 1];
    const float4 q2 = reinterpret_cast<const float4*>(gacc)[3 * (size_t)i + 2];
    dm2[0] = (0.5f * (float)sc.width * INV_LOG2E) * q0.x;
    dm2[1] = (0.5f * (float)sc.height * INV_LOG2E) * q0.y;
    const float dcon[3] = {-0.5f * q0.z, -0.5f * q0.w, -0.5f * q1.x};
    dop = q1.y;
    const float ddep = q1.z;
    dcol[0] = q2.x; dcol[1] = q2.y; dcol[2] = q2.z;
    clamp_bits = __float_as_uint(reinterpret_cast<const float4*>(cx.geom + i)[2].w) >> 29;

    if (wrow) {
      skin = skin_position(sc, i, wrow);
      p = skin.world;
    } else {
      p = make_float3(__ldg(sc.means3D + 3 * (size_t)i), __ldg(sc.means3D + 3 * (size_t)i + 1),
                      __ldg(sc.means3D + 3 * (size_t)i + 2));
    }
    float c6[6];
    float3 scl = make_float3(0.f, 0.f, 0.f);
    float4 q = make_float4(1.f, 0.f, 0.f, 0.f);
    if (sc.cov3D_precomp) {
#pragma unroll
      for (int k = 0; k < 6; k++) c6[k] = __ldg(sc.cov3D_precomp + 6 * (size_t)i + k);
    } else {
      scl = make_float3(__ldg(sc.scales + 3 * (size_t)i), __ldg(sc.scales + 3 * (size_t)i + 1),
                        __ldg(sc.scales + 3 * (size_t)i + 2));
      const float* qp = sc.rotations + 4 * (size_t)i;
      q = make_float4(__ldg(qp), __ldg(qp + 1), __ldg(qp + 2), __ldg(qp + 3));
      cov3d_from_scale_rot(scl, sc.scale_modifier, q, c6);
    }
    const float3 pv = xform4x3(p, cam.v);
    Ewa e;
    ewa_project(pv, c6, cam, e);

    const float a = e.a, b = e.b, c = e.c;
    const float denom = a * c - b * b;
    const float d2inv = 1.f / (denom * denom + K_EPS_W);
    float dLa = 0.f, dLb = 0.f, dLc = 0.f;
    if (d2inv != 0.f) {
      dLa = d2inv * (-c * c * dcon[0] + 2.f * b * c * dcon[1] + (denom - a * c) * dcon[2]);
      dLc = d2inv * (-a * a * dcon[2] + 2.f * a * b * dcon[1] + (denom - a * c) * dcon[0]);
      dLb = d2inv * 2.f * (b * c * dcon[0] - (denom + 2.f * b * b) * dcon[1] + a * b * dcon[2]);
      const float* A0 = e.A0;
      const float* A1 = e.A1;
      dS[0] = A0[0] * A0[0] * dLa + A0[0] * A1[0] * dLb + A1[0] * A1[0] * dLc;
      dS[3] = A0[1] * A0[1] * dLa + A0[1] * A1[1] * dLb + A1[1] * A1[1] * dLc;
      dS[5] = A0[2] * A0[2] * dLa + A0[2] * A1[2] * dLb + A1[2] * A1[2] * dLc;
      dS[1] = 2.f * A0[0] * A0[1] * dLa + (A0[0] * A1[1] + A0[1] * A1[0]) * dLb + 2.f * A1[0] * A1[1] * dLc;
      dS[2] = 2.f * A0[0] * A0[2] * dLa + (A0[0] * A1[2] + A0[2] * A1[0]) * dLb + 2.f * A1[0] * A1[2] * dLc;
      dS[4] = 2.f * A0[2] * A0[1] * dLa + (A0[1] * A1[2] + A0[2] * A1[1]) * dLb + 2.f * A1[1] * A1[2] * dLc;
    }
    const float S[9] = {c6[0], c6[1], c6[2], c6[1], c6[3], c6[4], c6[2], c6[4], c6[5]};
    float dA0[3], dA1[3];
#pragma unroll
    for (int k = 0; k < 3; k++) {
      const float SA0 = e.A0[0] * S[3 * k] + e.A0[1] * S[3 * k + 1] + e.A0[2] * S[3 * k + 2];
      const float SA1 = e.A1[0] * S[3 * k] + e.A1[1] * S[3 * k + 1] + e.A1[2] * S[3 * k + 2];
      dA0[k] = 2.f * SA0 * dLa + SA1 * dLb;
      dA1[k] = 2.f * SA1 * dLc + SA0 * dLb;
    }
    const float* v = cam.v;
    const float dJ00 = dA0[0] * v[0] + dA0[1] * v[4] + dA0[2] * v[8];
    const float dJ02 = dA0[0] * v[2] + dA0[1] * v[6] + dA0[2] * v[10];
    const float dJ11 = dA1[0] * v[1] + dA1[1] * v[5] + dA1[2] * v[9];
    const float dJ12 = dA1[0] * v[2] + dA1[1] * v[6] + dA1[2] * v[10];
    const float tz = 1.f / e.t[2], tz2 = tz * tz, tz3 = tz2 * tz;
    const float dtx = e.xmul * -cam.fx * tz2 * dJ02;
    const float dty = e.ymul * -cam.fy * tz2 * dJ12;
    const float dtz = -cam.fx * tz2 * dJ00 - cam.fy * tz2 * dJ11 + (2.f * cam.fx * e.t[0]) * tz3 * dJ02 +
                      (2.f * cam.fy * e.t[1]) * tz3 * dJ12;
    dm[0] = v[0] * dtx + v[1] * dty + v[2] * dtz;
    dm[1] = v[4] * dtx + v[5] * dty + v[6] * dtz;
    dm[2] = v[8] * dtx + v[9] * dty + v[10] * dtz;

    const float* pm = cam.p;
    const float4 mh = xform4x4(p, pm);
    const float mw = 1.f / (mh.w + K_EPS_W);
    const float mul1 = mh.x * mw * mw, mul2 = mh.y * mw * mw;
    dm[0] += (pm[0] * mw - pm[3] * mul1) * dm2[0] + (pm[1] * mw - pm[3] * mul2) * dm2[1];
    dm[1] += (pm[4] * mw - pm[7] * mul1) * dm2[0] + (pm[5] * mw - pm[7] * mul2) * dm2[1];
    dm[2] += (pm[8] * mw - pm[11] * mul1) * dm2[0] + (pm[9] * mw - pm[11] * mul2) * dm2[1];
    dm[0] += v[2] * ddep;
    dm[1] += v[6] * ddep;
    dm[2] += v[10] * ddep;

    if (!sc.cov3D_precomp) {
      float R[9];
      quat_to_R(q, R);
      const float mod = sc.scale_modifier;
      const float s[3] = {mod * scl.x, mod * scl.y, mod * scl.z};
      const float G3[9] = {dS[0], 0.5f * dS[1], 0.5f * dS[2], 0.5f * dS[1], dS[3], 0.5f * dS[4], 0.5f * dS[2], 0.5f * dS[4], dS[5]};
      float dR[9];
#pragma unroll
      for (int k = 0; k < 3; k++) {
        float dN[3];
#pragma unroll
        for (int r = 0; r < 3; r++)
          dN[r] = 2.f * (G3[3 * r] * R[k] * s[k] + G3[3 * r + 1] * R[3 + k] * s[k] + G3[3 * r + 2] * R[6 + k] * s[k]);
        dscale[k] = mod * (R[k] * dN[0] + R[3 + k] * dN[1] + R[6 + k] * dN[2]);
#pragma unroll
        for (int r = 0; r < 3; r++) dR[3 * r + k] = dN[r] * s[k];
      }
      const float r = q.x, x = q.y, y = q.z, z = q.w;
      dq[0] = 2.f * (-z * dR[1] + y * dR[2] + z * dR[3] - x * dR[5] - y * dR[6] + x * dR[7]);
      dq[1] = 2.f * (y * dR[1] + z * dR[2] + y * dR[3] - 2.f * x * dR[4] - r * dR[5] + z * dR[6] + r * dR[7] - 2.f * x * dR[8]);
      dq[2] = 2.f * (-2.f * y * dR[0] + x * dR[1] + r * dR[2] + x * dR[3] + z * dR[5] - r * dR[6] + z * dR[7] - 2.f * y * dR[8]);
      dq[3] = 2.f * (-2.f * z * dR[0] - r * dR[1] + x * dR[2] + r * dR[3] - 2.f * z * dR[4] + y * dR[5] + x * dR[6] + y * dR[7]);
    }
  }

  if (shrow) {
    if (!visible) {
      for (int k = 0; k < M * 3; k++) shrow[k] = 0.f;
    } else {
      const int deg = sc.sh_degree;
      const int used = (deg + 1) * (deg + 1);
      const float ddx = p.x - cam.campos[0], ddy = p.y - cam.campos[1], ddz = p.z - cam.campos[2];
      const float n = sqrtf(ddx * ddx + ddy * ddy + ddz * ddz);
      const float x = ddx / n, y = ddy / n, z = ddz / n;
      const float xx = x * x, yy = y * y, zz = z * z, xy = x * y, yz = y * z, xz = x * z;
      float ddir[3] = {0.f, 0.f, 0.f};
#pragma unroll
      for (int c = 0; c < 3; c++) {
        const float gc = ((clamp_bits >> c) & 1u) ? 0.f : dcol[c];
        float shv[16];
#pragma unroll
        for (int k = 0; k < 16; k++) shv[k] = k < used ? shrow[k * 3 + c] : 0.f;
        auto SH = [&](int k) { return shv[k]; };
        auto DSH = [&](int k, float basis) { shrow[k * 3 + c] = basis * gc; };
        float drx = 0.f, dry = 0.f, drz = 0.f;
        DSH(0, B2R_SH_C0);
        if (deg > 0) {
          DSH(1, -B2R_SH_C1 * y); DSH(2, B2R_SH_C1 * z); DSH(3, -B2R_SH_C1 * x);
          drx += -B2R_SH_C1 * SH(3); dry += -B2R_SH_C1 * SH(1); drz += B2R_SH_C1 * SH(2);
          if (deg > 1) {
            DSH(4, c_SH_C2[0] * xy); DSH(5, c_SH_C2[1] * yz); DSH(6, c_SH_C2[2] * (2.f * zz - xx - yy));
            DSH(7, c_SH_C2[3] * xz); DSH(8, c_SH_C2[4] * (xx - yy));
            drx += c_SH_C2[0] * y * SH(4) - 2.f * c_SH_C2[2] * x * SH(6) + c_SH_C2[3] * z * SH(7) + 2.f * c_SH_C2[4] * x * SH(8);
            dry += c_SH_C2[0] * x * SH(4) + c_SH_C2[1] * z * SH(5) - 2.f * c_SH_C2[2] * y * SH(6) - 2.f * c_SH_C2[4] * y * SH(8);
            drz += c_SH_C2[1] * y * SH(5) + 4.f * c_SH_C2[2] * z * SH(6) + c_SH_C2[3] * x * SH(7);
            if (deg > 2) {
              DSH(9, c_SH_C3[0] * y * (3.f * xx - yy));
              DSH(10, c_SH_C3[1] * xy * z);
              DSH(11, c_SH_C3[2] * y * (4.f * zz - xx - yy));
              DSH(12, c_SH_C3[3] * z * (2.f * zz - 3.f * xx - 3.f * yy));
              DSH(13, c_SH_C3[4] * x * (4.f * zz - xx - yy));
              DSH(14, c_SH_C3[5] * z * (xx - yy));
              DSH(15, c_SH_C3[6] * x * (xx - 3.f * yy));
              drx += c_SH_C3[0] * SH(9) * 6.f * xy + c_SH_C3[1] * SH(10) * yz - c_SH_C3[2] * SH(11) * 2.f * xy -
                     c_SH_C3[3] * SH(12) * 6.f * xz + c_SH_C3[4] * SH(13) * (4.f * zz - 3.f * xx - yy) +
                     c_SH_C3[5] * SH(14) * 2.f * xz + c_SH_C3[6] * SH(15) * 3.f * (xx - yy);
              dry += c_SH_C3[0] * SH(9) * 3.f * (xx - yy) + c_SH_C3[1] * SH(10) * xz +
                     c_SH_C3[2] * SH(11) * (4.f * zz - xx - 3.f * yy) - c_SH_C3[3] * SH(12) * 6.f * yz -
                     c_SH_C3[4] * SH(13) * 2.f * xy - c_SH_C3[5] * SH(14) * 2.f * yz - c_SH_C3[6] * SH(15) * 6.f * xy;
              drz += c_SH_C3[1] * SH(10) * xy + c_SH_C3[2] * SH(11) * 8.f * yz +
                     c_SH_C3[3] * SH(12) * 3.f * (2.f * zz - xx - yy) + c_SH_C3[4] * SH(13) * 8.f * xz +
                     c_SH_C3[5] * SH(14) * (xx - yy);
            }
          }
        }
        for (int k = used; k < M; k++) shrow[k * 3 + c] = 0.f;
        ddir[0] += drx * gc;
        ddir[1] += dry * gc;
        ddir[2] += drz * gc;
      }
      const float dot = x * ddir[0] + y * ddir[1] + z * ddir[2];
      dm[0] += (ddir[0] - x * dot) / n;
      dm[1] += (ddir[1] - y * dot) / n;
      dm[2] += (ddir[2] - z * dot) / n;
    }
  }

  if (posed_in) {
    dm[0] += __ldg(out.dL_dposed + 3 * (size_t)i);
    dm[1] += __ldg(out.dL_dposed + 3 * (size_t)i + 1);
    dm[2] += __ldg(out.dL_dposed + 3 * (size_t)i + 2);
  }
  const bool track = visible && (out.densify_rows == 0u || (uint32_t)i < out.densify_rows);
  if (track && out.densify_grad_accum) out.densify_grad_accum[oi] += sqrtf(dm2[0] * dm2[0] + dm2[1] * dm2[1]);
  if (track && out.densify_count) out.densify_count[oi] += 1.f;
  if (track && out.densify_radius_max) out.densify_radius_max[oi] = fmaxf(out.densify_radius_max[oi], (float)aux.z);
  auto put3 = [&](float* base, const float* v) {
    if (!base) return;
    float* d = base + 3 * oi;
    if (accumulate) { d[0] += v[0]; d[1] += v[1]; d[2] += v[2]; }
    else { d[0] = v[0]; d[1] = v[1]; d[2] = v[2]; }
  };
  if (wrow && (out.dL_dskin_xyz || out.dL_dskin_G)) {
    float gc[3] = {dm[0], dm[1], dm[2]}, dx[3] = {0.f, 0.f, 0.f}, G[12];
    float xs[4] = {0.f, 0.f, 0.f, 0.f};
    if (visible || posed_in) {
      skin_transpose(skin.M, sc.skin_cam_Rinv, dm, gc, dx);
      xs[0] = skin.x.x; xs[1] = skin.x.y; xs[2] = skin.x.z; xs[3] = 1.f;
    }
#pragma unroll
    for (int r = 0; r < 3; r++)
#pragma unroll
      for (int c = 0; c < 4; c++) G[4 * r + c] = gc[r] * xs[c];
    put3(out.dL_dskin_xyz, dx);
    if (out.dL_dskin_G) {
      float* d = out.dL_dskin_G + 12 * oi;
#pragma unroll
      for (int k = 0; k < 12; k++) { if (accumulate) d[k] += G[k]; else d[k] = G[k]; }
    }
  }
  const float dm2z[3] = {dm2[0], dm2[1], 0.f};
  put3(out.dL_dmeans3D, dm);
  put3(out.dL_dmeans2D, dm2z);
  if (MIXED && shrow) {
    const float zero3[3] = {0.f, 0.f, 0.f};
    put3(out.dL_dcolors, zero3);
  } else {
    put3(out.dL_dcolors, dcol);
  }
  put3(out.dL_dscales, dscale);
  if (out.dL_dopacities) {
    if (accumulate) out.dL_dopacities[oi] += dop; else out.dL_dopacities[oi] = dop;
  }
  if (out.dL_drotations) {
#pragma unroll
    for (int k = 0; k < 4; k++) {
      float* d = out.dL_drotations + 4 * oi + k;
      if (accumulate) *d += dq[k]; else *d = dq[k];
    }
  }
  if (out.dL_dcov3D) {
#pragma unroll
    for (int k = 0; k < 6; k++) {
      float* d = out.dL_dcov3D + 6 * oi + k;
      const float v = sc.cov3D_precomp ? dS[k] : 0.f;
      if (accumulate) *d += v; else *d = v;
    }
  }
}

#ifndef PBWD_MIN_BLOCKS
#define PBWD_MIN_BLOCKS 3
#endif
template <bool MIXED>
__global__ void __launch_bounds__(256, PBWD_MIN_BLOCKS) project_bwd_kernel(const B2RScene sc, const Ctx cx, const B2RBackwardArgs out,
                                                          const float* __restrict__ gacc) {
  extern __shared__ float sh_stage[];
  const int i = blockIdx.x * blockDim.x + threadIdx.x;
  const int lane = threadIdx.x & 31, warp = threadIdx.x >> 5;
  const bool in_range = i < sc.P;
  const bool accumulate = (out.flags & B2R_BWD_ACCUMULATE) != 0;
  int4 aux = make_int4(0, 0, 0, 0);
  if (in_range) aux = cx.aux[i];
  const bool visible = aux.z > 0;
  const int first_row = (int)out.first_row;
  const bool active = in_range && i >= first_row && !(accumulate && !visible && out.dL_dposed == nullptr);
  const bool use_sh = sc.shs != nullptr && out.dL_dshs != nullptr;
  const int L = sc.sh_coeffs * 3, S = L | 1;
  float* wstage = sh_stage + (size_t)warp * 32 * S;
  const int row0 = blockIdx.x * blockDim.x + warp * 32;
  const int nrows = min(32, sc.P - row0);
  const int sh_nrows = MIXED ? min(32, sc.sh_rows - row0) : nrows;
  if (use_sh && sh_nrows > 0) {
    stage_rows<0>(wstage, const_cast<float*>(sc.shs) + (size_t)row0 * L, L, sh_nrows, 0xffffffffu);
    __syncwarp();
  }
  float* shrow = use_sh && (!MIXED || i < sc.sh_rows) ? wstage + lane * S : nullptr;
  const float* wrow = nullptr;
  if (sc.skin_xyz) {
    const int J = sc.skin_J, SJ = J | 1;
    float* kstage = sh_stage + (use_sh ? (size_t)8 * 32 * S : 0) + (size_t)warp * 32 * SJ;
    if (nrows > 0) stage_rows<0>(kstage, const_cast<float*>(sc.skin_weights) + (size_t)row0 * J, J, nrows, 0xffffffffu);
    __syncwarp();
    wrow = kstage + lane * SJ;
  }
  if (active) project_bwd_one<MIXED>(sc, cx, out, gacc, i, (size_t)(i - first_row), visible, aux, shrow, wrow);
  if ((out.flags & B2R_BWD_SCRATCH_ZEROED) && in_range && visible) {
    float4* row = reinterpret_cast<float4*>(const_cast<float*>(gacc)) + 3 * (size_t)i;
    row[0] = row[1] = row[2] = make_float4(0.f, 0.f, 0.f, 0.f);
  }
  if (use_sh && sh_nrows > 0) {
    const unsigned rows_active = __ballot_sync(0xffffffffu, active && (!MIXED || i < sc.sh_rows));
    __syncwarp();
    float* dst = out.dL_dshs + ((ptrdiff_t)row0 - first_row) * L;
    if (accumulate) stage_rows<2>(wstage, dst, L, sh_nrows, rows_active);
    else stage_rows<1>(wstage, dst, L, sh_nrows, rows_active);
  }
}

int launch_project_bwd(const B2RScene& sc, const Ctx& cx, const B2RBackwardArgs& a, const float* gacc, cudaStream_t st) {
  ProfScope p(K_PROJECT_BWD, st, sc.P > 0 ? 1 : 0);
  if (sc.P > 0) {
    const bool use_sh = sc.shs != nullptr && a.dL_dshs != nullptr;
    const size_t smem = (use_sh ? (size_t)8 * 32 * ((sc.sh_coeffs * 3) | 1) * sizeof(float) : 0) +
                        (sc.skin_xyz ? (size_t)8 * 32 * (sc.skin_J | 1) * sizeof(float) : 0);
    auto kern = sc.sh_rows > 0 ? project_bwd_kernel<true> : project_bwd_kernel<false>;
    cudaFuncSetAttribute(kern, cudaFuncAttributeMaxDynamicSharedMemorySize, 128 * 1024);
    launch_k(kern, (sc.P + 255) / 256, 256, smem, st, true, sc, cx, a, gacc);
  }
  return check_launch();
}

}
```

exavatar_release_b200/plan.py:

```python
from __future__ import annotations

import ctypes as C
import os
from typing import Dict, Optional

import torch

from . import _lib as L
from .rasterizer import _f32c, _make_scene, _ptr


class _Workspace:

    def __init__(self, P: int, width: int, height: int, dup_capacity: int, device, checkpoints: bool = True):
        self.lib = L.load()
        self.P, self.W, self.H = int(P), int(width), int(height)
        self.device = dev = torch.device(device)
        self.capacity = int(dup_capacity)
        self.radii = torch.empty(P, dtype=torch.int32, device=dev)
        self.ctx_bytes = self.lib.b2r_ctx_bytes(P, width, height)
        self.ctx_buf = torch.empty(self.ctx_bytes, dtype=torch.uint8, device=dev)
        self.ids = torch.empty(max(self.capacity, 1), dtype=torch.int32, device=dev)
        self.scratch_bytes = self.lib.b2r_scratch_bytes(P, width, height, self.capacity)
        self.scratch = torch.empty(self.scratch_bytes, dtype=torch.uint8, device=dev)
        self.bwd_bytes = self.lib.b2r_backward_scratch_bytes(P)
        self.bwd_scratch = torch.zeros(self.bwd_bytes, dtype=torch.uint8, device=dev)
        self.ckpt_bytes = self.lib.b2r_checkpoint_bytes(width, height, self.capacity) if checkpoints else 0
        self.ckpt = torch.empty(max(self.ckpt_bytes, 1), dtype=torch.uint8, device=dev) if checkpoints else None
        self.ws = L.B2RWorkspace(self.ctx_buf.data_ptr(), self.ctx_bytes, self.ids.data_ptr(), self.capacity,
                                 self.scratch.data_ptr(), self.scratch_bytes, None, 0,
                                 self.ckpt.data_ptr() if checkpoints else None, self.ckpt_bytes)

    def status(self) -> dict:
        return L.read_status(self.ctx_buf)


class FramePlan(_Workspace):
    def __init__(self, P: int, width: int, height: int, dup_capacity: int, device, sh_coeffs: int = 0,
                 segmented: bool = True):
        segmented = segmented and os.environ.get("B2R_SEGMENTED", "1") != "0"
        super().__init__(P, width, height, dup_capacity, device, checkpoints=segmented)
        self.M = int(sh_coeffs)
        f = lambda *s: torch.empty(s, dtype=torch.float32, device=self.device)
        self.color, self.depth, self.alpha = f(3, height, width), f(1, height, width), f(1, height, width)
        self.out = L.B2RForwardOutputs(self.color.data_ptr(), self.depth.data_ptr(), self.alpha.data_ptr(),
                                       self.radii.data_ptr())
        self._scenes = {}
        self._primed = False

    def scene(self, key, settings, assets: Dict[str, torch.Tensor], flags: int = 0):
        if key in self._scenes:
            return self._scenes[key][0]
        g = lambda k: None if assets.get(k) is None else _f32c(assets[k], k)
        shs = g("shs") if self.M > 0 else None
        sc, keep = _make_scene(settings, g("mean_3d"), shs, None if shs is not None else g("rgb"), g("opacity"),
                               g("scale"), g("rotation"), None, flags)
        self._scenes[key] = (sc, keep)
        return sc

    def forward(self, sc) -> None:
        base = sc.flags & ~L.B2R_FLAG_CTX_CLEAN
        sc.flags = base | (L.B2R_FLAG_CTX_CLEAN if self._primed else 0)
        with torch.cuda.device(self.device):
            st = torch.cuda.current_stream(self.device).cuda_stream
            L.check(self.lib.b2r_forward(C.byref(sc), C.byref(self.ws), C.byref(self.out), st), "b2r_forward")
        sc.flags = base
        self._primed = True

    def backward(self, sc, g_color: torch.Tensor, grads: Dict[str, Optional[torch.Tensor]], accumulate: bool = False,
                 g_depth: Optional[torch.Tensor] = None, g_alpha: Optional[torch.Tensor] = None,
                 densify: Optional[Dict[str, torch.Tensor]] = None, first_row: int = 0) -> None:
        a = L.B2RBackwardArgs(_ptr(g_color), _ptr(g_depth), _ptr(g_alpha), _ptr(grads.get("means3D")),
                              _ptr(grads.get("means2D")), _ptr(grads.get("shs")), _ptr(grads.get("colors")),
                              _ptr(grads.get("opacities")), _ptr(grads.get("scales")), _ptr(grads.get("rotations")),
                              _ptr(grads.get("cov3D")), (L.B2R_BWD_ACCUMULATE if accumulate else 0) | L.B2R_BWD_SCRATCH_ZEROED, int(first_row),
                              _ptr((densify or {}).get("grad_accum")), _ptr((densify or {}).get("count")),
                              _ptr((densify or {}).get("radius_max")))
        with torch.cuda.device(self.device):
            st = torch.cuda.current_stream(self.device).cuda_stream
            L.check(self.lib.b2r_backward(C.byref(sc), C.byref(self.ws), C.byref(a), self.bwd_scratch.data_ptr(),
                                          self.bwd_bytes, st), "b2r_backward")


def grad_bucket(P: int, device, sh_coeffs: int = 0):
    per = 3 + 3 + 1 + 3 + 4 + (3 * sh_coeffs if sh_coeffs > 0 else 3)
    return _views_of(torch.zeros(per * P, dtype=torch.float32, device=device), P, sh_coeffs)


class FrameLanes:

    def __init__(self, lanes: int, P: int, width: int, height: int, dup_capacity: int, device, sh_coeffs: int = 0):
        self.S = max(1, int(lanes))
        self.device = torch.device(device)
        self.plans = [FramePlan(P, width, height, dup_capacity, device, sh_coeffs) for _ in range(self.S)]
        self.streams = [torch.cuda.Stream(self.device) for _ in range(self.S)]
        flat0, _ = grad_bucket(P, device, sh_coeffs)
        self.lane_flat = torch.zeros(self.S, flat0.numel(), dtype=torch.float32, device=device)
        self.lane_views = []
        for s in range(self.S):
            _, v = _views_of(self.lane_flat[s], P, sh_coeffs)
            self.lane_views.append(v)
        self.bucket = self.lane_flat[0] if self.S == 1 else flat0
        _, self.views = _views_of(self.bucket, P, sh_coeffs)

    def scene(self, key, settings, assets, flags: int = 0):
        return self.plans[0].scene(key, settings, assets, flags)

    def step(self, scenes, g_colors, backward: bool = True) -> None:
        cur = torch.cuda.current_stream(self.device)
        F = len(scenes)
        for s in range(self.S):
            st = self.streams[s]
            st.wait_stream(cur)
            with torch.cuda.stream(st):
                plan = self.plans[s]
                for j, f in enumerate(range(s, F, self.S)):
                    plan.forward(scenes[f])
                    if backward:
                        plan.backward(scenes[f], g_colors[f], self.lane_views[s], accumulate=(j > 0))
        for st in self.streams:
            cur.wait_stream(st)
        if backward and self.S > 1:
            torch.sum(self.lane_flat[: min(self.S, F)], dim=0, out=self.bucket)

    def status(self) -> dict:
        sts = [p.status() for p in self.plans]
        out = dict(sts[0])
        out["overflow"] = int(any(s["overflow"] for s in sts))
        return out


def _views_of(flat: torch.Tensor, P: int, sh_coeffs: int = 0):
    widths = [("means3D", 3), ("means2D", 3), ("opacities", 1), ("scales", 3), ("rotations", 4)]
    widths.append(("shs", 3 * sh_coeffs) if sh_coeffs > 0 else ("colors", 3))
    views, o = {}, 0
    for name, w in widths:
        views[name] = flat[o:o + w * P].view(P, w) if name != "shs" else flat[o:o + w * P].view(P, sh_coeffs, 3)
        o += w * P
    return flat, views


RENDERS = ("scene", "human", "scene_human", "human_refined", "scene_human_refined")


class FiveRenderPlan:
    PER = 3 + 3 + 1 + 3 + 4 + 3

    def __init__(self, P_scene: int, P_human: int, width: int, height: int, caps: Optional[Dict[str, int]], device):
        self.Ps, self.Ph = int(P_scene), int(P_human)
        self.device = torch.device(device)
        caps = caps or {r: 8_000_000 for r in RENDERS}
        sizes = {"scene": self.Ps, "human": self.Ph, "scene_human": self.Ps + self.Ph, "human_refined": self.Ph,
                 "scene_human_refined": self.Ps + self.Ph}
        self.plans = {r: FramePlan(sizes[r], width, height, caps[r], device) for r in RENDERS}
        self.streams = {r: torch.cuda.Stream(self.device) for r in RENDERS}
        self.first_row = {"scene": 0, "human": 0, "scene_human": self.Ps, "human_refined": 0, "scene_human_refined": self.Ps}
        out_rows = {"scene": self.Ps, "human": self.Ph, "scene_human": self.Ph, "human_refined": self.Ph,
                    "scene_human_refined": self.Ph}
        order = ("scene", "human", "human_refined", "scene_human", "scene_human_refined")
        tail = 2 * self.Ps
        self.all_flat = torch.zeros(self.PER * sum(out_rows[r] for r in order) + tail, dtype=torch.float32, device=device)
        self.flat, self.views, o = {}, {}, 0
        for r in order:
            n = self.PER * out_rows[r]
            self.flat[r], self.views[r] = _views_of(self.all_flat[o:o + n], out_rows[r])
            o += n
            if r == "human_refined":
                self._stats = self.all_flat[o:o + tail]
                o += tail
        self._reduced = self.PER * (self.Ps + 2 * self.Ph) + tail
        f = lambda w: torch.empty(self.Ps + self.Ph, w, dtype=torch.float32, device=device)
        widths = {"mean_3d": 3, "opacity": 1, "scale": 3, "rotation": 4, "rgb": 3}
        self.cat = {r: {k: f(w) for k, w in widths.items()} for r in ("scene_human", "scene_human_refined")}

    def describe(self) -> str:
        return "five independent renders (project+bin+sort+composite each) on five CUDA streams per frame"

    def set_scene(self, scene_assets: Dict[str, torch.Tensor]) -> None:
        for r in self.cat:
            for k, buf in self.cat[r].items():
                buf[: self.Ps].copy_(scene_assets[k].reshape(self.Ps, -1))

    def assets_of(self, render: str, scene, human, refined):
        if render == "scene":
            return scene
        if render in ("human", "human_refined"):
            return human if render == "human" else refined
        src = human if render == "scene_human" else refined
        for k, buf in self.cat[render].items():
            buf[self.Ps:].copy_(src[k].reshape(self.Ph, -1))
        return self.cat[render]

    def frame(self, key, settings, settings_human_bg, scene, human, refined, g_colors: Dict[str, torch.Tensor],
              accumulate: bool, densify: Optional[Dict[str, torch.Tensor]] = None, serial: bool = False) -> None:
        cur = torch.cuda.current_stream(self.device)
        for r in RENDERS:
            st = cur if serial else self.streams[r]
            if not serial:
                st.wait_stream(cur)
            with torch.cuda.stream(st):
                plan = self.plans[r]
                assets = self.assets_of(r, scene, human, refined)
                sc = plan.scene((key, r), settings_human_bg if r in ("human", "human_refined") else settings, assets)
                plan.forward(sc)
                plan.backward(sc, g_colors[r], self.views[r], accumulate=accumulate, first_row=self.first_row[r],
                              densify=densify if r == "scene" else None)
        if not serial:
            for r in RENDERS:
                cur.wait_stream(self.streams[r])

    def render_outputs(self, render: str):
        p = self.plans[render]
        return p.color, p.alpha, p.radii

    def reduce(self):
        self.flat["human"].add_(self.flat["scene_human"])
        self.flat["human_refined"].add_(self.flat["scene_human_refined"])
        return self.flat["scene"], self.flat["human"], self.flat["human_refined"]

    def grads(self, which: str) -> Dict[str, torch.Tensor]:
        return dict(self.views[which])

    def flat_bucket(self) -> torch.Tensor:
        return self.all_flat[: self._reduced]

    def stats(self) -> Dict[str, torch.Tensor]:
        return {"grad_accum": self._stats[: self.Ps], "count": self._stats[self.Ps:]}

    def zero_stats(self) -> None:
        self._stats.zero_()

    def dups(self) -> Dict[str, int]:
        return {r: p.status()["num_dups"] for r, p in self.plans.items()}

    def consumed(self) -> Dict[str, list]:
        st = [self.plans[r].status() for r in RENDERS]
        return {"fwd": [s["consumed_fwd"] / s["consumed_fwd_div"] for s in st],
                "bwd": [s["consumed_bwd"] / s["consumed_bwd_div"] for s in st]}

    def overflowed(self) -> bool:
        return any(p.status()["overflow"] for p in self.plans.values())


class _Pass(_Workspace):

    def __init__(self, P, W, H, cap, n_views, device):
        super().__init__(P, W, H, cap, device)
        dev = self.device
        self.ck = [self.ckpt] + [torch.empty_like(self.ckpt) for _ in range(n_views - 1)]
        f = lambda *s: torch.empty(s, dtype=torch.float32, device=dev)
        self.img = [(f(3, H, W), f(1, H, W), f(1, H, W)) for _ in range(n_views)]
        self.state = [(f(H * W), torch.empty(H * W, dtype=torch.int32, device=dev)) for _ in range(n_views)]
        widths = {"mean_3d": 3, "opacity": 1, "scale": 3, "rotation": 4, "rgb": 3}
        self.cat = {k: f(P, w) for k, w in widths.items()}
        self.streams = [torch.cuda.Stream(dev) for _ in range(n_views)]
        self.primed = False


def merged_bucket_layout(P_scene: int, P_human: int, sh_coeffs: int = 0) -> Dict[str, tuple]:
    PER = FiveRenderPlan.PER
    Ps, Ph, M = int(P_scene), int(P_human), int(sh_coeffs)
    nA, nS, nB = PER * (Ps + Ph), 3 * M * Ps, PER * Ph
    return {"A": (0, nA), "A_shs": (nA, nS), "B": (nA + nS, nB), "stats": (nA + nS + nB, 2 * Ps),
            "total": (0, nA + nS + nB + 2 * Ps)}


def merged_pass_a_views(flat: torch.Tensor, P_scene: int, P_human: int, sh_coeffs: int = 0) -> Dict[str, torch.Tensor]:
    lay = merged_bucket_layout(P_scene, P_human, sh_coeffs)
    (oa, na), (os_, ns) = lay["A"], lay["A_shs"]
    _, views = _views_of(flat[oa:oa + na], int(P_scene) + int(P_human))
    if sh_coeffs > 0:
        views["shs"] = flat[os_:os_ + ns].view(int(P_scene), int(sh_coeffs), 3)
    return views


class MergedFivePlan:
    PER = FiveRenderPlan.PER
    VIEWS = {"A": ("scene", "human", "scene_human"), "B": ("human_refined", "scene_human_refined")}
    SKIP = os.environ.get("B2R_SKIP_TILES", "1") != "0"

    def __init__(self, P_scene: int, P_human: int, width: int, height: int, caps: Optional[Dict[str, int]], device,
                 sh_coeffs: int = 0):
        self.lib = L.load()
        self.Ps, self.Ph, self.P = int(P_scene), int(P_human), int(P_scene) + int(P_human)
        self.W, self.H = int(width), int(height)
        self.M = int(sh_coeffs)
        self.device = torch.device(device)
        caps = caps or {"A": 8_000_000, "B": 8_000_000}
        self.passes = {k: _Pass(self.P, self.W, self.H, caps[k], len(v), self.device) for k, v in self.VIEWS.items()}
        self.pass_streams = {k: torch.cuda.Stream(self.device) for k in self.passes}
        lay = merged_bucket_layout(self.Ps, self.Ph, self.M)
        self.all_flat = torch.zeros(lay["total"][1], dtype=torch.float32, device=device)
        o, n = lay["stats"]
        self._stats = self.all_flat[o:o + n]
        self.views_A = merged_pass_a_views(self.all_flat, self.Ps, self.Ph, self.M)
        o, n = lay["B"]
        _, self.views_B = _views_of(self.all_flat[o:o + n], self.Ph)
        self.shs = torch.zeros(self.Ps, self.M, 3, dtype=torch.float32, device=device) if self.M > 0 else None
        self._shs_src, self.sh_degree = self.shs, 0
        Ps, P = self.Ps, self.P
        self.ranges = {"scene": (0, Ps), "human": (Ps, P), "scene_human": (0, P), "human_refined": (Ps, P),
                       "scene_human_refined": (0, P)}
        self.first_row = {"scene": 0, "human": Ps, "scene_human": Ps, "human_refined": Ps, "scene_human_refined": Ps}
        self._scenes = {}
        self._current = {}
        self._keep = []

    def describe(self) -> str:
        return ("two merged passes per frame (cat(scene,human): 3 views; cat(scene,refined): 2 views), each one "
                "projection + binning + sort; composites of a pass on parallel CUDA streams")

    def set_scene(self, scene_assets: Dict[str, torch.Tensor]) -> None:
        for ps in self.passes.values():
            for k, buf in ps.cat.items():
                if k == "rgb" and self.M > 0:
                    continue
                buf[: self.Ps].copy_(scene_assets[k].reshape(self.Ps, -1))
        if self.M > 0:
            self.use_scene_shs(scene_assets["shs"], scene_assets["sh_degree"])

    def use_scene_shs(self, shs: torch.Tensor, sh_degree: int, copy: bool = False) -> None:
        if self.M == 0:
            raise ValueError("MergedFivePlan: built without SH (sh_coeffs=0); pass the scene colours as `rgb`")
        t = shs.detach()
        if tuple(t.shape) != (self.Ps, self.M, 3):
            raise ValueError(f"MergedFivePlan: scene `shs` must be ({self.Ps}, {self.M}, 3), got {tuple(t.shape)}")
        if copy or t.dtype != torch.float32 or not t.is_contiguous() or t.device != self.device:
            self.shs.copy_(t)
            t = self.shs
        self._shs_src, self.sh_degree = t, int(sh_degree)

    def _scene_desc(self, key, ps, settings):
        def make():
            shs = self._shs_src if self.M > 0 else None
            sc, keep = _make_scene(settings, ps.cat["mean_3d"], shs, ps.cat["rgb"], ps.cat["opacity"], ps.cat["scale"],
                                   ps.cat["rotation"], None, 0)
            if shs is not None:
                sc.sh_rows, sc.sh_degree = self.Ps, self.sh_degree
            return sc, keep

        if key[0] is None:
            sc, keep = make()
            ps.last_scene = (sc, keep)
            return sc
        if self.M > 0:
            key = (key, self._shs_src.data_ptr(), self.sh_degree)
        if key not in self._scenes:
            self._scenes[key] = make()
        return self._scenes[key][0]

    def _human_bg(self, settings_human_bg) -> torch.Tensor:
        bg_h = _f32c(settings_human_bg.bg.to(self.device), "bg")
        self._keep.append(bg_h)
        del self._keep[:-64]
        return bg_h

    def _view(self, ps, v, name, bg):
        lo, hi = self.ranges[name]
        fT, nc = ps.state[v]
        skip = self.Ps if (self.SKIP and name != "scene") else 0
        return L.B2RView(lo, hi, _ptr(bg), fT.data_ptr(), nc.data_ptr(), ps.ck[v].data_ptr(), ps.ckpt_bytes, skip, 0)

    def _start_pass(self, s, pk, key, settings, src, bg_h) -> None:
        ps = self.passes[pk]
        if src is not None:
            for k, buf in ps.cat.items():
                buf[self.Ps:].copy_(src[k].reshape(self.Ph, -1))
        sc = self._scene_desc((key, pk), ps, settings)
        sc.flags = L.B2R_FLAG_CTX_CLEAN if ps.primed else 0
        ps.primed = True
        L.check(self.lib.b2r_forward_project(C.byref(sc), C.byref(ps.ws), ps.radii.data_ptr(), s.cuda_stream),
                "b2r_forward_project")
        L.check(self.lib.b2r_forward_bin(C.byref(sc), C.byref(ps.ws), s.cuda_stream), "b2r_forward_bin")
        views = [self._view(ps, v, n, bg_h if n in ("human", "human_refined") else None)
                 for v, n in enumerate(self.VIEWS[pk])]
        self._current[pk] = (sc, views)

    def _forward_view(self, s, pk, v, bg_h, scene_done) -> None:
        ps, name = self.passes[pk], self.VIEWS[pk][v]
        sc, views = self._current[pk]
        color, depth, alpha = ps.img[v]
        if views[v].skip_below and name in ("human", "human_refined"):
            color.copy_(bg_h.view(3, 1, 1).expand_as(color))
            depth.zero_()
            alpha.zero_()
        elif views[v].skip_below:
            s.wait_event(scene_done)
            for dst, src in zip(ps.img[v], self.passes["A"].img[0]):
                dst.copy_(src)
        out = L.B2RForwardOutputs(color.data_ptr(), depth.data_ptr(), alpha.data_ptr(), ps.radii.data_ptr())
        L.check(self.lib.b2r_forward_composite(C.byref(sc), C.byref(ps.ws), C.byref(views[v]), C.byref(out),
                                               s.cuda_stream), "b2r_forward_composite")
        if name == "scene":
            scene_done.record(s)

    def _backward_view(self, s, pk, v, g_color, g_depth=None, g_alpha=None) -> None:
        ps = self.passes[pk]
        sc, views = self._current[pk]
        a = L.B2RBackwardArgs(_ptr(g_color), _ptr(g_depth), _ptr(g_alpha))
        a.flags = L.B2R_BWD_SCRATCH_ZEROED
        a.first_row = self.first_row[self.VIEWS[pk][v]]
        L.check(self.lib.b2r_backward_composite(C.byref(sc), C.byref(ps.ws), C.byref(views[v]), C.byref(a),
                                                ps.bwd_scratch.data_ptr(), ps.bwd_bytes, s.cuda_stream),
                "b2r_backward_composite")

    def _backward_project(self, s, pk, g, accumulate, densify) -> None:
        ps = self.passes[pk]
        sc, _ = self._current[pk]
        a = L.B2RBackwardArgs(None, None, None, _ptr(g["means3D"]), _ptr(g["means2D"]),
                              _ptr(g.get("shs")) if pk == "A" else None, _ptr(g["colors"]),
                              _ptr(g["opacities"]), _ptr(g["scales"]), _ptr(g["rotations"]), None)
        a.flags = (L.B2R_BWD_ACCUMULATE if accumulate else 0) | L.B2R_BWD_SCRATCH_ZEROED
        a.first_row = 0 if pk == "A" else self.Ps
        if pk == "A" and densify is not None:
            a.densify_grad_accum, a.densify_count = _ptr(densify.get("grad_accum")), _ptr(densify.get("count"))
            a.densify_radius_max = _ptr(densify.get("radius_max"))
            a.densify_rows = self.Ps
        L.check(self.lib.b2r_backward_project(C.byref(sc), C.byref(ps.ws), C.byref(a), ps.bwd_scratch.data_ptr(),
                                              ps.bwd_bytes, s.cuda_stream), "b2r_backward_project")

    def frame(self, key, settings, settings_human_bg, scene, human, refined, g_colors: Dict[str, torch.Tensor],
              accumulate: bool, densify: Optional[Dict[str, torch.Tensor]] = None, serial: bool = False, probe=None) -> None:
        probe = probe if (probe is not None and serial) else (lambda label: None)
        cur = torch.cuda.current_stream(self.device)
        bg_h = self._human_bg(settings_human_bg)
        scene_done = torch.cuda.Event()
        for pk, names in self.VIEWS.items():
            ps = self.passes[pk]
            st = cur if serial else self.pass_streams[pk]
            if not serial:
                st.wait_stream(cur)
            with torch.cuda.stream(st):
                self._start_pass(st, pk, key, settings, human if pk == "A" else refined, bg_h)
                probe(f"{pk}:bin")
                for v, n in enumerate(names):
                    vs = st if serial else ps.streams[v]
                    if not serial:
                        vs.wait_stream(st)
                    with torch.cuda.stream(vs):
                        self._forward_view(vs, pk, v, bg_h, scene_done)
                        probe(f"{pk}:{n}:fwd")
                        self._backward_view(vs, pk, v, g_colors[n])
                        probe(f"{pk}:{n}:bwd")
                if not serial:
                    for v in range(len(names)):
                        st.wait_stream(ps.streams[v])
                self._backward_project(st, pk, self.views_A if pk == "A" else self.views_B, accumulate, densify)
                probe(f"{pk}:project_bwd")
        if not serial:
            for pk in self.passes:
                cur.wait_stream(self.pass_streams[pk])

    def forward_frame(self, key, settings, settings_human_bg, scene, human, refined, copy_inputs: bool = True) -> None:
        cur = torch.cuda.current_stream(self.device)
        bg_h = self._human_bg(settings_human_bg)
        scene_done = torch.cuda.Event()
        for pk, names in self.VIEWS.items():
            ps = self.passes[pk]
            st = self.pass_streams[pk]
            st.wait_stream(cur)
            with torch.cuda.stream(st):
                src = (human if pk == "A" else refined) if copy_inputs else None
                self._start_pass(st, pk, key, settings, src, bg_h)
                for v in range(len(names)):
                    vs = ps.streams[v]
                    vs.wait_stream(st)
                    with torch.cuda.stream(vs):
                        self._forward_view(vs, pk, v, bg_h, scene_done)
                for v in range(len(names)):
                    st.wait_stream(ps.streams[v])
        for pk in self.passes:
            cur.wait_stream(self.pass_streams[pk])

    def backward_frame(self, g_colors: Dict[str, Optional[torch.Tensor]], grads_A: Dict[str, torch.Tensor],
                       grads_B: Dict[str, torch.Tensor], g_depths: Optional[Dict[str, torch.Tensor]] = None,
                       g_alphas: Optional[Dict[str, torch.Tensor]] = None, accumulate: bool = False,
                       densify: Optional[Dict[str, torch.Tensor]] = None) -> None:
        cur = torch.cuda.current_stream(self.device)
        for pk, names in self.VIEWS.items():
            ps = self.passes[pk]
            st = self.pass_streams[pk]
            st.wait_stream(cur)
            with torch.cuda.stream(st):
                for v, n in enumerate(names):
                    gc, gd, ga = g_colors.get(n), (g_depths or {}).get(n), (g_alphas or {}).get(n)
                    if gc is None and gd is None and ga is None:
                        continue
                    vs = ps.streams[v]
                    vs.wait_stream(st)
                    with torch.cuda.stream(vs):
                        if gc is None:
                            gc = torch.zeros(3, self.H, self.W, dtype=torch.float32, device=self.device)
                        self._backward_view(vs, pk, v, gc, gd, ga)
                        self._keep.append((gc, gd, ga))
                for v in range(len(names)):
                    st.wait_stream(ps.streams[v])
                self._backward_project(st, pk, grads_A if pk == "A" else grads_B, accumulate, densify)
        for pk in self.passes:
            cur.wait_stream(self.pass_streams[pk])

    def render_outputs(self, render: str):
        pk = "A" if render in self.VIEWS["A"] else "B"
        ps = self.passes[pk]
        color, _, alpha = ps.img[self.VIEWS[pk].index(render)]
        lo, hi = self.ranges[render]
        return color, alpha, ps.radii[lo:hi]

    def reduce(self):
        return self.grads("scene"), self.grads("human"), self.grads("human_refined")

    def grads(self, which: str) -> Dict[str, torch.Tensor]:
        if which == "scene":
            out = {k: v[: self.Ps] for k, v in self.views_A.items() if k != "shs"}
            if self.M > 0:
                del out["colors"]
                out["shs"] = self.views_A["shs"]
            return out
        if which == "human":
            return {k: v[self.Ps:] for k, v in self.views_A.items() if k != "shs"}
        return dict(self.views_B)

    def flat_bucket(self) -> torch.Tensor:
        return self.all_flat

    def stats(self) -> Dict[str, torch.Tensor]:
        return {"grad_accum": self._stats[: self.Ps], "count": self._stats[self.Ps:]}

    def zero_stats(self) -> None:
        self._stats.zero_()

    def dups(self) -> Dict[str, int]:
        return {k: ps.status()["num_dups"] for k, ps in self.passes.items()}

    def consumed(self) -> Dict[str, list]:
        fwd, bwd = [], []
        for pk, names in self.VIEWS.items():
            s = self.passes[pk].status()
            fwd += [s["consumed_fwd"] / L.CONSUMED_FWD_DIV / len(names)] * len(names)
            bwd += [s["consumed_bwd"] / L.CONSUMED_BWD_DIV / len(names)] * len(names)
        return {"fwd": fwd, "bwd": bwd}

    def overflowed(self) -> bool:
        return any(ps.status()["overflow"] for ps in self.passes.values())
```

include/b200raster.h:

```cpp
#ifndef B200RASTER_H_
#define B200RASTER_H_

#include <stddef.h>
#include <stdint.h>

#ifdef __cplusplus
extern "C" {
#endif

#define B2R_ABI_VERSION 3

#define B2R_OK 0
#define B2R_E_INVALID (-1)
#define B2R_E_WORKSPACE (-2)
#define B2R_E_CUDA (-3)
#define B2R_E_DUP_OVERFLOW (-4)

#define B2R_FLAG_NO_TILE_CULL 1u
#define B2R_FLAG_DEBUG 2u
#define B2R_FLAG_CTX_CLEAN 4u

typedef struct B2RScene {
  int32_t P;
  int32_t width, height;
  int32_t sh_degree;
  int32_t sh_coeffs;
  uint32_t flags;
  float scale_modifier;
  float tanfovx, tanfovy;
  const float* bg;
  const float* viewmatrix;
  const float* projmatrix;
  const float* campos;
  const float* means3D;
  const float* shs;
  const float* colors_precomp;
  const float* opacities;
  const float* scales;
  const float* rotations;
  const float* cov3D_precomp;
  const float* skin_xyz;
  const float* skin_weights;
  const float* skin_joint_mats;
  const float* skin_trans;
  const float* skin_cam_Rinv;
  const float* skin_cam_t;
  float* skin_means_out;
  int32_t skin_J;
  int32_t sh_rows;
} B2RScene;

typedef struct B2RStatus {
  uint64_t num_dups;
  uint64_t dup_capacity;
  uint32_t overflow;
  uint32_t num_visible;
  uint64_t consumed_fwd;
  uint64_t consumed_bwd;
  uint64_t token;
  uint64_t reserved[2];
} B2RStatus;

typedef struct B2RWorkspace {
  void* ctx;
  size_t ctx_bytes;
  uint32_t* dup_ids;
  uint64_t dup_capacity;
  void* scratch;
  size_t scratch_bytes;
  uint64_t* status_mirror;
  uint64_t status_token;
  void* checkpoints;
  size_t checkpoint_bytes;
} B2RWorkspace;

typedef struct B2RView {
  uint32_t id_begin, id_end;
  const float* bg;
  float* final_T;
  uint32_t* n_contrib;
  void* checkpoints;
  size_t checkpoint_bytes;
  uint32_t skip_below;
  uint32_t reserved;
} B2RView;

typedef struct B2RForwardOutputs {
  float* color;
  float* depth;
  float* alpha;
  int32_t* radii;
} B2RForwardOutputs;

typedef struct B2RBackwardArgs {
  const float* dL_dcolor;
  const float* dL_ddepth;
  const float* dL_dalpha;
  float* dL_dmeans3D;
  float* dL_dmeans2D;
  float* dL_dshs;
  float* dL_dcolors;
  float* dL_dopacities;
  float* dL_dscales;
  float* dL_drotations;
  float* dL_dcov3D;
  uint32_t flags;
  uint32_t first_row;
  float* densify_grad_accum;
  float* densify_count;
  float* densify_radius_max;
  float* dL_dskin_xyz;
  float* dL_dskin_G;
  const float* dL_dposed;
  uint32_t densify_rows;
  uint32_t reserved;
} B2RBackwardArgs;
typedef struct B2RSkin {
  int32_t P;
  int32_t J;
  int32_t V;
  int32_t reserved;
  const float* weights;
  const int32_t* rows;
  const float* joint_mats;
  const float* trans;
  const float* cam_Rinv;
  const float* cam_t;
  const float* xyz[2];
  float* posed[2];
} B2RSkin;

#define B2R_BWD_ACCUMULATE 1u
#define B2R_BWD_SCRATCH_ZEROED 2u

int b2r_abi_version(void);
const char* b2r_strerror(int code);
int b2r_last_cuda_error(void);
size_t b2r_sizeof(int which);

size_t b2r_ctx_bytes(int32_t P, int32_t width, int32_t height);
size_t b2r_scratch_bytes(int32_t P, int32_t width, int32_t height, uint64_t dup_capacity);
size_t b2r_backward_scratch_bytes(int32_t P);
size_t b2r_checkpoint_bytes(int32_t width, int32_t height, uint64_t dup_capacity);

int b2r_forward_project(const B2RScene* scene, const B2RWorkspace* ws, int32_t* radii, void* stream);
int b2r_forward_render(const B2RScene* scene, const B2RWorkspace* ws, const B2RForwardOutputs* out, void* stream);
int b2r_forward(const B2RScene* scene, const B2RWorkspace* ws, const B2RForwardOutputs* out, void* stream);

int b2r_backward(const B2RScene* scene, const B2RWorkspace* ws, const B2RBackwardArgs* args, void* bwd_scratch,
                 size_t bwd_scratch_bytes, void* stream);

int b2r_forward_bin(const B2RScene* scene, const B2RWorkspace* ws, void* stream);
int b2r_forward_composite(const B2RScene* scene, const B2RWorkspace* ws, const B2RView* view,
                          const B2RForwardOutputs* out, void* stream);
int b2r_backward_composite(const B2RScene* scene, const B2RWorkspace* ws, const B2RView* view, const B2RBackwardArgs* args,
                           void* bwd_scratch, size_t bwd_scratch_bytes, void* stream);
int b2r_backward_project(const B2RScene* scene, const B2RWorkspace* ws, const B2RBackwardArgs* args, void* bwd_scratch,
                         size_t bwd_scratch_bytes, void* stream);

int b2r_skin_forward(const B2RSkin* skin, void* stream);
int b2r_skin_backward(const B2RSkin* skin, const float* const dL_dposed[2], float* const dL_dxyz[2], float* dL_djoint,
                      float* dL_dtrans, void* scratch, size_t scratch_bytes, void* stream);
size_t b2r_skin_scratch_bytes(int32_t P, int32_t J);

size_t b2r_l1ssim_scratch_bytes(int32_t width, int32_t height);
int b2r_l1ssim_forward(int32_t width, int32_t height, const float* img, const float* target, const float* mask,
                       const float* bbox, int32_t with_ssim, float* out, void* scratch, size_t scratch_bytes,
                       void* stream);
int b2r_l1ssim_backward(int32_t width, int32_t height, const float* img, const float* target, const float* mask,
                        const float* bbox, int32_t with_ssim, const float* dL_dout, float* dL_dimg, const void* scratch,
                        size_t scratch_bytes, void* stream);

size_t b2r_nearest_scratch_bytes(int32_t P, int32_t V);
int b2r_nearest_rows(int32_t P, const float* queries, int32_t V, const float* targets, const uint8_t* self_map,
                     int32_t* rows, void* scratch, size_t scratch_bytes, void* stream);

int b2r_vertex_normals(int32_t P, const float* xyz, const int32_t* faces, const int32_t* vf_offsets,
                       const int32_t* vf_entries, const uint8_t* flip, float* normals, void* stream);

typedef struct B2RMeshRender {
  int32_t V;
  int32_t F;
  int32_t Vt;
  int32_t C;
  int32_t tex_height, tex_width;
  int32_t height, width;
  const float* mesh;
  const int32_t* faces;
  const float* vertex_uv;
  const int32_t* face_uv;
  const float* texture;
  const float* cam_R;
  const float* cam_t;
  const float* focal;
  const float* princpt;
  uint64_t* keys;
  const int32_t* vf_offsets;
  const int32_t* vf_entries;
} B2RMeshRender;

size_t b2r_mesh_render_scratch_bytes(int32_t F);
int b2r_mesh_render_forward(const B2RMeshRender* mr, float* image, int32_t* pix_to_face, void* scratch,
                            size_t scratch_bytes, void* stream);
int b2r_mesh_render_backward(const B2RMeshRender* mr, const int32_t* pix_to_face, const float* dL_dimage,
                             float* dL_dmesh, void* scratch, size_t scratch_bytes, void* stream);

int b2r_mark_visible(int32_t P, const float* means3D, const float* viewmatrix, uint8_t* present, void* stream);

#define B2R_NUM_KERNELS 9
void b2r_profile_enable(int on);
int b2r_profile_read(double* ms_sum, uint64_t* counts, int reset);
uint64_t b2r_launch_count(void);
const char* b2r_kernel_name(int id);

const float* b2r_ctx_geom(const B2RWorkspace* ws, int32_t P, int32_t width, int32_t height);
const int32_t* b2r_ctx_aux(const B2RWorkspace* ws, int32_t P, int32_t width, int32_t height);
const uint32_t* b2r_ctx_ranges(const B2RWorkspace* ws, int32_t P, int32_t width, int32_t height);
const float* b2r_ctx_final_T(const B2RWorkspace* ws, int32_t P, int32_t width, int32_t height);
const uint32_t* b2r_ctx_n_contrib(const B2RWorkspace* ws, int32_t P, int32_t width, int32_t height);

#ifdef __cplusplus
}
#endif
#endif
```

Measured before the change: 1600.

## Reuse pass A scene binning in refined pass via split project, sort and merge

Pass B (refined human views) shares the scene Gaussians with pass A. It now projects and scatters only the human rows. It copies the scene rows' geometry and radii from pass A, sorts only its own per-tile keys, and merges them with pass A's already depth-sorted scene ids per tile using a rank-by-binary-search merge. This avoids re-projecting and re-sorting the scene Gaussians. In exchange, pass B must wait on pass A's binning event, which reduces overlap between the two passes, and it adds prepare and merge kernels.

```diff
diff --git a/exavatar_release_b200/_lib.py b/exavatar_release_b200/_lib.py
--- a/exavatar_release_b200/_lib.py
+++ b/exavatar_release_b200/_lib.py
@@ -118,6 +118,10 @@
     ("b2r_backward_project", C.c_int, [C.POINTER(B2RScene), C.POINTER(B2RWorkspace), C.POINTER(B2RBackwardArgs), _fp,
                                        C.c_size_t, _fp]),
     ("b2r_forward_project", C.c_int, [C.POINTER(B2RScene), C.POINTER(B2RWorkspace), _fp, _fp]),
+    ("b2r_split_scratch_bytes", C.c_size_t, [C.c_int32, C.c_int32, C.c_int32, C.c_uint64]),
+    ("b2r_forward_project_split", C.c_int, [C.POINTER(B2RScene), C.POINTER(B2RWorkspace), C.c_uint32, _fp, _fp]),
+    ("b2r_forward_bin_split", C.c_int, [C.POINTER(B2RScene), C.POINTER(B2RWorkspace), C.POINTER(B2RWorkspace),
+                                        C.c_uint32, _fp, _fp]),
     ("b2r_forward_render", C.c_int, [C.POINTER(B2RScene), C.POINTER(B2RWorkspace), C.POINTER(B2RForwardOutputs), _fp]),
     ("b2r_forward", C.c_int, [C.POINTER(B2RScene), C.POINTER(B2RWorkspace), C.POINTER(B2RForwardOutputs), _fp]),
     ("b2r_backward", C.c_int, [C.POINTER(B2RScene), C.POINTER(B2RWorkspace), C.POINTER(B2RBackwardArgs), _fp,
diff --git a/exavatar_release_b200/csrc/api.cu b/exavatar_release_b200/csrc/api.cu
--- a/exavatar_release_b200/csrc/api.cu
+++ b/exavatar_release_b200/csrc/api.cu
@@ -184,6 +184,43 @@
   return launch_binning(*scene, cx, false, (cudaStream_t)stream);
 }
 
+size_t b2r_split_scratch_bytes(int32_t P, int32_t width, int32_t height, uint64_t dup_capacity) {
+  return split_scratch_bytes(P, width, height, dup_capacity);
+}
+
+int b2r_forward_project_split(const B2RScene* scene, const B2RWorkspace* ws, uint32_t first_row, int32_t* radii,
+                              void* stream) {
+  int rc = validate_scene(scene);
+  if (rc) return rc;
+  rc = validate_ws(scene, ws, false);
+  if (rc) return rc;
+  if ((int64_t)first_row > (int64_t)scene->P) return B2R_E_INVALID;
+  if (ws->dup_capacity == 0) return B2R_E_INVALID;
+  if (scene->P > 0 && !radii) return B2R_E_INVALID;
+  const Ctx cx = resolve(ws, scene->P, scene->width, scene->height);
+  return launch_project(*scene, cx, radii, (cudaStream_t)stream, (int)first_row);
+}
+
+int b2r_forward_bin_split(const B2RScene* scene, const B2RWorkspace* ws, const B2RWorkspace* base, uint32_t first_row,
+                          int32_t* radii, void* stream) {
+  int rc = validate_scene(scene);
+  if (rc) return rc;
+  rc = validate_ws(scene, ws, true);
+  if (rc) return rc;
+  if ((int64_t)first_row > (int64_t)scene->P) return B2R_E_INVALID;
+  if (ws->dup_capacity == 0 || (scene->P > 0 && !radii)) return B2R_E_INVALID;
+  if (ws->scratch_bytes < split_scratch_bytes(scene->P, scene->width, scene->height, ws->dup_capacity))
+    return B2R_E_WORKSPACE;
+  if (!base || base == ws || !base->ctx || !base->dup_ids) return B2R_E_INVALID;
+  if (base->ctx_bytes < b2r_ctx_bytes(scene->P, scene->width, scene->height)) return B2R_E_WORKSPACE;
+  Ctx cx = resolve(ws, scene->P, scene->width, scene->height);
+  cx.sort_len = (uint32_t*)((char*)ws->ctx + ctx_layout(scene->P, scene->width, scene->height).split_len);
+  const Ctx bx = resolve(base, scene->P, scene->width, scene->height);
+  uint32_t* own_ids = (uint32_t*)((char*)ws->scratch + scratch_layout(scene->P, scene->width, scene->height,
+                                                                      ws->dup_capacity).total);
+  return launch_binning_split(*scene, cx, bx, own_ids, (int)first_row, radii, (cudaStream_t)stream);
+}
+
 int b2r_forward_composite(const B2RScene* scene, const B2RWorkspace* ws, const B2RView* view,
                           const B2RForwardOutputs* out, void* stream) {
   int rc = validate_scene(scene);
diff --git a/exavatar_release_b200/csrc/binning.cu b/exavatar_release_b200/csrc/binning.cu
--- a/exavatar_release_b200/csrc/binning.cu
+++ b/exavatar_release_b200/csrc/binning.cu
@@ -4,8 +4,8 @@
 
 namespace b2r {
 
-__global__ void __launch_bounds__(256) scatter_kernel(const B2RScene sc, const Ctx cx) {
-  const int i = blockIdx.x * blockDim.x + threadIdx.x;
+__global__ void __launch_bounds__(256) scatter_kernel(const B2RScene sc, const Ctx cx, const int first_row) {
+  const int i = first_row + blockIdx.x * blockDim.x + threadIdx.x;
   int4 aux = make_int4(0, 0, 0, 0);
   float4 g0 = make_float4(0.f, 0.f, 0.f, 0.f), g1 = g0;
   uint32_t depth_bits = 0u;
@@ -35,13 +35,13 @@
   if (pend_pos < cap) keys[pend_pos] = make_uint2(pend_depth, pend_id);
 }
 
-__global__ void __launch_bounds__(256) scatter_agg_kernel(const B2RScene sc, const Ctx cx) {
+__global__ void __launch_bounds__(256) scatter_agg_kernel(const B2RScene sc, const Ctx cx, const int first_row) {
   extern __shared__ uint32_t s_mem[];
   uint32_t* s_cnt = s_mem;
   uint32_t* s_base = s_mem + cx.tiles;
   for (int t = threadIdx.x; t < cx.tiles; t += blockDim.x) s_cnt[t] = 0u;
   __syncthreads();
-  const int i = blockIdx.x * blockDim.x + threadIdx.x;
+  const int i = first_row + blockIdx.x * blockDim.x + threadIdx.x;
   int4 aux = make_int4(0, 0, 0, 0);
   float4 g0 = make_float4(0.f, 0.f, 0.f, 0.f), g1 = g0;
   uint32_t depth_bits = 0u;
@@ -408,14 +408,14 @@
       const uint32_t tile = cx.tile_order[lo];
       const uint2 r = cx.ranges[tile];
       const int off = (b - (int)cx.chunk_start[lo]) * SORT_CHUNK;
-      const int len = min(SORT_CHUNK, (int)(r.y - r.x) - off);
+      const int len = min(SORT_CHUNK, sort_length(cx, (int)tile, r) - off);
       if (len > 1) radix_sort_tile<CAP, THREADS, true>(cx.keys + r.x + off, nullptr, len, smem_raw, cx.tile_maxid + tile);
       else if (len == 1 && threadIdx.x == 0) atomicMax(cx.tile_maxid + tile, cx.keys[r.x + off].y);
       last_n = len;
     } else if (b < n_chunks + n_cta) {
       const uint32_t tile = cx.tile_order[n_large + (b - n_chunks)];
       const uint2 r = cx.ranges[tile];
-      const int n = (int)(r.y - r.x);
+      const int n = sort_length(cx, (int)tile, r);
       const uint2* src = cx.keys + r.x;
       uint32_t* dst = cx.dup_ids + r.x;
       if (n > 32) {
@@ -431,9 +431,9 @@
       if (t < cx.tiles) {
         const uint32_t tile = cx.tile_order[t];
         const uint2 r = cx.ranges[tile];
-        last_n = -(int)(r.y - r.x);
-        warp_sort_tile(cx.keys + r.x, cx.dup_ids + r.x, (int)(r.y - r.x), smem_raw + (size_t)warp * WSORT_BYTES,
-                       cx.tile_maxid + tile);
+        const int n = sort_length(cx, (int)tile, r);
+        last_n = -n;
+        warp_sort_tile(cx.keys + r.x, cx.dup_ids + r.x, n, smem_raw + (size_t)warp * WSORT_BYTES, cx.tile_maxid + tile);
       }
     }
   }
@@ -459,8 +459,9 @@
       const int cs = mid < n_tab ? (int)table[mid] : (int)cx.chunk_start[mid];
       if (cs <= b) lo = mid; else hi = mid - 1;
     }
-    const uint2 r = cx.ranges[cx.tile_order[lo]];
-    const int n = (int)(r.y - r.x);
+    const uint32_t tile = cx.tile_order[lo];
+    const uint2 r = cx.ranges[tile];
+    const int n = sort_length(cx, (int)tile, r);
     const int c = b - (int)(lo < n_tab ? table[lo] : cx.chunk_start[lo]);
     const uint2* pairs = cx.keys + r.x;
     const int chunks = (n + SORT_CHUNK - 1) / SORT_CHUNK;
@@ -520,6 +521,7 @@
 }
 
 constexpr int SORT_SMALL = SORT_CHUNK;
+void launch_sort(const Ctx& cx, cudaStream_t st);
 
 int launch_binning(const B2RScene& sc, const Ctx& cx, bool rescan, cudaStream_t st) {
   if (rescan) {
@@ -532,11 +534,16 @@
     const size_t smem = (size_t)cx.tiles * 8;
     if (cx.tiles <= 2048) {
       cudaFuncSetAttribute(scatter_agg_kernel, cudaFuncAttributeMaxDynamicSharedMemorySize, 96 * 1024);
-      launch_k(scatter_agg_kernel, (sc.P + 255) / 256, 256, smem, st, true, sc, cx);
+      launch_k(scatter_agg_kernel, (sc.P + 255) / 256, 256, smem, st, true, sc, cx, 0);
     } else {
-      launch_k(scatter_kernel, (sc.P + 255) / 256, 256, 0, st, true, sc, cx);
-    }
-  }
+      launch_k(scatter_kernel, (sc.P + 255) / 256, 256, 0, st, true, sc, cx, 0);
+    }
+  }
+  launch_sort(cx, st);
+  return check_launch();
+}
+
+void launch_sort(const Ctx& cx, cudaStream_t st) {
   const int sms = device_sm_count();
   constexpr int ST = 256;
   constexpr size_t cta_bytes = RadixSmem<SORT_SMALL, ST>::bytes, warp_bytes = (ST / 32) * WSORT_BYTES;
@@ -550,6 +557,137 @@
     ProfScope p(K_SORT_LARGE, st);
     launch_k(merge_chunks_kernel, 2 * sms, 256, 0, st, true, cx);
   }
+}
+
+
+__global__ void __launch_bounds__(256) split_prepare_kernel(const Ctx cx, const Ctx base, const int split,
+                                                            int32_t* __restrict__ radii) {
+  const int tid = threadIdx.x;
+  const float4* gsrc = reinterpret_cast<const float4*>(base.geom);
+  float4* gdst = reinterpret_cast<float4*>(cx.geom);
+  for (size_t k = (size_t)blockIdx.x * 256 + tid; k < (size_t)split * 3; k += (size_t)gridDim.x * 256) gdst[k] = gsrc[k];
+  for (int k = blockIdx.x * 256 + tid; k < split; k += gridDim.x * 256) radii[k] = base.aux[k].z;
+  for (int t = blockIdx.x; t < cx.tiles; t += gridDim.x) {
+    const uint32_t own = cx.tile_count[t];
+    uint32_t s = 0;
+    if (own) {
+      const uint2 rb = base.ranges[t];
+      for (uint32_t k = rb.x; k < rb.y; k += 256)
+        s += (uint32_t)__syncthreads_count(k + tid < rb.y && base.dup_ids[k + tid] < (uint32_t)split);
+    }
+    if (tid == 0) {
+      cx.sort_len[t] = own;
+      cx.tile_count[t] = own + s;
+    }
+    __syncthreads();
+  }
+}
+
+constexpr int SPLIT_CHUNK = 2048;
+constexpr int SPLIT_PER = 8;
+__global__ void __launch_bounds__(256) split_merge_kernel(const Ctx cx, const Ctx base, const uint32_t* __restrict__ own_ids,
+                                                          const int split) {
+  __shared__ uint2 other[SPLIT_CHUNK];
+  __shared__ uint32_t wtot[8];
+  const int tid = threadIdx.x, lane = tid & 31, warp = tid >> 5;
+  const uint32_t tile = cx.tile_order[blockIdx.x];
+  const uint2 r = cx.ranges[tile];
+  const int n = (int)(r.y - r.x);
+  if (n == 0) return;
+  const int n_own = sort_length(cx, (int)tile, r);
+  uint2* keys = cx.keys + r.x;
+  for (int i = tid; i < n_own; i += 256) {
+    const uint32_t id = own_ids[r.x + i];
+    keys[i] = make_uint2(__float_as_uint(cx.geom[id].g1.z), id);
+  }
+  const uint2 rb = base.ranges[tile];
+  int n_base = 0;
+  for (uint32_t k0 = rb.x; k0 < rb.y; k0 += 256) {
+    const uint32_t k = k0 + tid;
+    const uint32_t id = k < rb.y ? base.dup_ids[k] : 0xffffffffu;
+    const bool take = id < (uint32_t)split;
+    const unsigned b = __ballot_sync(0xffffffffu, take);
+    if (lane == 0) wtot[warp] = __popc(b);
+    __syncthreads();
+    int off = n_base, tot = 0;
+    for (int w = 0; w < 8; w++) {
+      off += w < warp ? (int)wtot[w] : 0;
+      tot += (int)wtot[w];
+    }
+    off += __popc(b & ((1u << lane) - 1u));
+    if (take && n_own + off < n) keys[n_own + off] = make_uint2(__float_as_uint(cx.geom[id].g1.z), id);
+    n_base += tot;
+    __syncthreads();
+  }
+  __syncthreads();
+  if (n_own + n_base != n) {
+    for (int i = tid; i < n; i += 256) cx.dup_ids[r.x + i] = keys[i].y;
+    return;
+  }
+  for (int side = 0; side < 2; side++) {
+    const uint2* mine = side ? keys + n_own : keys;
+    const uint2* oth = side ? keys : keys + n_own;
+    const int n_mine = side ? n_base : n_own, n_oth = side ? n_own : n_base;
+    for (int x0 = 0; x0 < n_mine; x0 += 256 * SPLIT_PER) {
+      unsigned long long key[SPLIT_PER];
+      int rank[SPLIT_PER];
+#pragma unroll
+      for (int j = 0; j < SPLIT_PER; j++) {
+        const int i = x0 + j * 256 + tid;
+        const uint2 v = i < n_mine ? mine[i] : make_uint2(0u, 0u);
+        key[j] = ((unsigned long long)v.x << 32) | v.y;
+        rank[j] = i;
+      }
+      for (int c0 = 0; c0 < n_oth; c0 += SPLIT_CHUNK) {
+        const int len2 = min(SPLIT_CHUNK, n_oth - c0);
+        __syncthreads();
+        for (int i = tid; i < len2; i += 256) other[i] = oth[c0 + i];
+        __syncthreads();
+#pragma unroll
+        for (int j = 0; j < SPLIT_PER; j++) {
+          int l = 0;
+          for (int step = SPLIT_CHUNK; step >= 1; step >>= 1) {
+            const int probe = l + step;
+            if (probe <= len2) {
+              const uint2 v = other[probe - 1];
+              if ((((unsigned long long)v.x << 32) | v.y) < key[j]) l = probe;
+            }
+          }
+          rank[j] += l;
+        }
+      }
+#pragma unroll
+      for (int j = 0; j < SPLIT_PER; j++)
+        if (x0 + j * 256 + tid < n_mine) cx.dup_ids[r.x + rank[j]] = (uint32_t)(key[j] & 0xffffffffull);
+    }
+  }
+}
+
+int launch_binning_split(const B2RScene& sc, const Ctx& cx_in, const Ctx& base, uint32_t* own_ids, const int first_row,
+                         int32_t* radii, cudaStream_t st) {
+  const Ctx& cx = cx_in;
+  {
+    ProfScope p(K_MISC, st);
+    launch_k(split_prepare_kernel, cx.tiles, 256, 0, st, true, cx, base, first_row, radii);
+  }
+  launch_tile_scan(cx, st, cx.dup_capacity > 0 ? 1 : 0);
+  if (sc.P > first_row) {
+    ProfScope p(K_SCATTER, st);
+    const unsigned grid = (unsigned)((sc.P - first_row + 255) / 256);
+    if (cx.tiles <= 2048) {
+      cudaFuncSetAttribute(scatter_agg_kernel, cudaFuncAttributeMaxDynamicSharedMemorySize, 96 * 1024);
+      launch_k(scatter_agg_kernel, grid, 256, (size_t)cx.tiles * 8, st, true, sc, cx, first_row);
+    } else {
+      launch_k(scatter_kernel, grid, 256, 0, st, true, sc, cx, first_row);
+    }
+  }
+  Ctx own = cx;
+  own.dup_ids = own_ids;
+  launch_sort(own, st);
+  {
+    ProfScope p(K_SORT_LARGE, st);
+    launch_k(split_merge_kernel, cx.tiles, 256, 0, st, true, cx, base, own_ids, first_row);
+  }
   return check_launch();
 }
 
diff --git a/exavatar_release_b200/csrc/common.cuh b/exavatar_release_b200/csrc/common.cuh
--- a/exavatar_release_b200/csrc/common.cuh
+++ b/exavatar_release_b200/csrc/common.cuh
@@ -52,7 +52,7 @@
 
 struct CtxLayout {
   size_t status, geom, aux, ranges, tile_count, tile_cursor, tile_order, chunk_start, seg_start, classes, tile_maxid,
-      final_T, n_contrib, total;
+      split_len, final_T, n_contrib, total;
   int gx, gy, tiles;
 };
 __host__ __device__ inline CtxLayout ctx_layout(int P, int W, int H) {
@@ -73,6 +73,7 @@
   L.seg_start = o; o += align_up((size_t)L.tiles * 4);
   L.classes = o; o += align_up((size_t)CLS_COUNT * 4);
   L.tile_maxid = o; o += align_up((size_t)L.tiles * 4);
+  L.split_len = o; o += align_up((size_t)L.tiles * 4);
   L.final_T = o; o += align_up(N * 4);
   L.n_contrib = o; o += align_up(N * 4);
   L.total = o;
@@ -89,6 +90,9 @@
   S.keys = o; o += align_up((size_t)(cap > 0 ? cap : 1) * 8);
   S.total = o;
   return S;
+}
+__host__ __device__ inline size_t split_scratch_bytes(int P, int W, int H, uint64_t cap) {
+  return scratch_layout(P, W, H, cap).total + align_up((size_t)(cap > 0 ? cap : 1) * 4);
 }
 
 struct Ctx {
@@ -117,7 +121,12 @@
   const float* bg;
   uint32_t* tile_maxid;
   uint32_t skip_below;
+  uint32_t* sort_len;
 };
+__device__ __forceinline__ int sort_length(const Ctx& cx, int tile, uint2 r) {
+  const int n = (int)(r.y - r.x);
+  return cx.sort_len ? min(n, (int)cx.sort_len[tile]) : n;
+}
 
 __host__ __device__ inline uint32_t max_segments(int tiles, uint64_t cap) { return (uint32_t)(cap / SEG) + (uint32_t)tiles; }
 __host__ __device__ inline size_t seg_table_bytes(uint32_t max_segs) { return align_up((size_t)max_segs * 8); }
@@ -159,6 +168,7 @@
   x.bg = nullptr;
   x.tile_maxid = (uint32_t*)(c + L.tile_maxid);
   x.skip_below = 0;
+  x.sort_len = nullptr;
   return x;
 }
 
@@ -419,9 +429,11 @@
   }
 }
 
-int launch_project(const B2RScene& sc, const Ctx& cx, int32_t* radii, cudaStream_t st);
+int launch_project(const B2RScene& sc, const Ctx& cx, int32_t* radii, cudaStream_t st, int first_row = 0);
 int launch_binning(const B2RScene& sc, const Ctx& cx, bool rescan, cudaStream_t st);
-void launch_tile_scan(const Ctx& cx, cudaStream_t st);
+int launch_binning_split(const B2RScene& sc, const Ctx& cx, const Ctx& base, uint32_t* own_ids, int first_row,
+                         int32_t* radii, cudaStream_t st);
+void launch_tile_scan(const Ctx& cx, cudaStream_t st, int final = 2);
 int launch_composite_fwd(const B2RScene& sc, const Ctx& cx, const B2RForwardOutputs& out, cudaStream_t st);
 int launch_composite_bwd(const B2RScene& sc, const Ctx& cx, const B2RBackwardArgs& a, float* gacc, cudaStream_t st);
 
diff --git a/exavatar_release_b200/csrc/project.cu b/exavatar_release_b200/csrc/project.cu
--- a/exavatar_release_b200/csrc/project.cu
+++ b/exavatar_release_b200/csrc/project.cu
@@ -39,19 +39,19 @@
 #endif
 template <bool MIXED>
 __global__ void __launch_bounds__(256, PROJ_MIN_BLOCKS) project_kernel(const B2RScene sc, const Ctx cx, int32_t* __restrict__ radii,
-                                                      const int aggregate) {
+                                                      const int aggregate, const int first_row) {
   extern __shared__ uint32_t s_cnt[];
   if (aggregate) {
     for (int t = threadIdx.x; t < cx.tiles; t += blockDim.x) s_cnt[t] = 0u;
     __syncthreads();
   }
-  const int i = blockIdx.x * blockDim.x + threadIdx.x;
+  const int i = first_row + blockIdx.x * blockDim.x + threadIdx.x;
   const float* shrow = nullptr;
   if (sc.shs) {
     const int lane = threadIdx.x & 31, warp = threadIdx.x >> 5;
     const int L = sc.sh_coeffs * 3, S = L | 1;
     float* wstage = reinterpret_cast<float*>(s_cnt + (aggregate ? cx.tiles : 0)) + (size_t)warp * 32 * S;
-    const int row0 = blockIdx.x * blockDim.x + warp * 32;
+    const int row0 = first_row + blockIdx.x * blockDim.x + warp * 32;
     const int nrows = min(32, (MIXED ? sc.sh_rows : sc.P) - row0);
     if (nrows > 0) stage_rows<0>(wstage, const_cast<float*>(sc.shs) + (size_t)row0 * L, L, nrows, 0xffffffffu);
     __syncwarp();
@@ -64,7 +64,7 @@
     float* base = reinterpret_cast<float*>(s_cnt + (aggregate ? cx.tiles : 0));
     if (sc.shs) base += (size_t)8 * 32 * ((sc.sh_coeffs * 3) | 1);
     float* wstage = base + (size_t)warp * 32 * S;
-    const int row0 = blockIdx.x * blockDim.x + warp * 32;
+    const int row0 = first_row + blockIdx.x * blockDim.x + warp * 32;
     const int nrows = min(32, sc.P - row0);
     if (nrows > 0) stage_rows<0>(wstage, const_cast<float*>(sc.skin_weights) + (size_t)row0 * J, J, nrows, 0xffffffffu);
     __syncwarp();
@@ -349,10 +349,10 @@
   present[i] = vz > K_NEAR ? 1 : 0;
 }
 
-int launch_project(const B2RScene& sc, const Ctx& cx, int32_t* radii, cudaStream_t st) {
+int launch_project(const B2RScene& sc, const Ctx& cx, int32_t* radii, cudaStream_t st, int first_row) {
   const bool clean = (sc.flags & B2R_FLAG_CTX_CLEAN) != 0;
   if (!clean) { ProfScope p(K_MISC, st); launch_k(status_reset_kernel, (cx.tiles + 1023) / 1024, 1024, 0, st, true, cx); }
-  if (sc.P > 0) {
+  if (sc.P > first_row) {
     ProfScope p(K_PROJECT, st);
     const int aggregate = cx.tiles <= 2048;
     const size_t smem = (aggregate ? (size_t)cx.tiles * 4 : 0) +
@@ -360,15 +360,18 @@
                         (sc.skin_xyz ? (size_t)8 * 32 * (sc.skin_J | 1) * sizeof(float) : 0);
     auto kern = sc.sh_rows > 0 ? project_kernel<true> : project_kernel<false>;
     cudaFuncSetAttribute(kern, cudaFuncAttributeMaxDynamicSharedMemorySize, 160 * 1024);
-    launch_k(kern, (sc.P + 255) / 256, 256, smem, st, true, sc, cx, radii, aggregate);
-  }
-  { ProfScope p(K_TILE_SCAN, st); launch_k(tile_scan_kernel, 1, 1024, 0, st, true, cx, cx.dup_capacity > 0 ? 1 : 0); }
+    launch_k(kern, (sc.P - first_row + 255) / 256, 256, smem, st, true, sc, cx, radii, aggregate, first_row);
+  }
+  if (first_row == 0) {
+    ProfScope p(K_TILE_SCAN, st);
+    launch_k(tile_scan_kernel, 1, 1024, 0, st, true, cx, cx.dup_capacity > 0 ? 1 : 0);
+  }
   return check_launch();
 }
 
-void launch_tile_scan(const Ctx& cx, cudaStream_t st) {
+void launch_tile_scan(const Ctx& cx, cudaStream_t st, int final) {
   ProfScope p(K_TILE_SCAN, st);
-  launch_k(tile_scan_kernel, 1, 1024, 0, st, true, cx, 2);
+  launch_k(tile_scan_kernel, 1, 1024, 0, st, true, cx, final);
 }
 
 int launch_mark_visible(int P, const float* means3D, const float* view, uint8_t* present, cudaStream_t st) {
diff --git a/exavatar_release_b200/csrc/project_bwd.cu b/exavatar_release_b200/csrc/project_bwd.cu
--- a/exavatar_release_b200/csrc/project_bwd.cu
+++ b/exavatar_release_b200/csrc/project_bwd.cu
@@ -265,7 +265,8 @@
 __global__ void __launch_bounds__(256, PBWD_MIN_BLOCKS) project_bwd_kernel(const B2RScene sc, const Ctx cx, const B2RBackwardArgs out,
                                                           const float* __restrict__ gacc) {
   extern __shared__ float sh_stage[];
-  const int i = blockIdx.x * blockDim.x + threadIdx.x;
+  const int blk = blockIdx.x + (int)out.first_row / 256;
+  const int i = blk * blockDim.x + threadIdx.x;
   const int lane = threadIdx.x & 31, warp = threadIdx.x >> 5;
   const bool in_range = i < sc.P;
   const bool accumulate = (out.flags & B2R_BWD_ACCUMULATE) != 0;
@@ -277,7 +278,7 @@
   const bool use_sh = sc.shs != nullptr && out.dL_dshs != nullptr;
   const int L = sc.sh_coeffs * 3, S = L | 1;
   float* wstage = sh_stage + (size_t)warp * 32 * S;
-  const int row0 = blockIdx.x * blockDim.x + warp * 32;
+  const int row0 = blk * blockDim.x + warp * 32;
   const int nrows = min(32, sc.P - row0);
   const int sh_nrows = MIXED ? min(32, sc.sh_rows - row0) : nrows;
   if (use_sh && sh_nrows > 0) {
@@ -308,14 +309,15 @@
 }
 
 int launch_project_bwd(const B2RScene& sc, const Ctx& cx, const B2RBackwardArgs& a, const float* gacc, cudaStream_t st) {
-  ProfScope p(K_PROJECT_BWD, st, sc.P > 0 ? 1 : 0);
-  if (sc.P > 0) {
+  const int grid = (sc.P + 255) / 256 - (int)a.first_row / 256;
+  ProfScope p(K_PROJECT_BWD, st, grid > 0 ? 1 : 0);
+  if (grid > 0) {
     const bool use_sh = sc.shs != nullptr && a.dL_dshs != nullptr;
     const size_t smem = (use_sh ? (size_t)8 * 32 * ((sc.sh_coeffs * 3) | 1) * sizeof(float) : 0) +
                         (sc.skin_xyz ? (size_t)8 * 32 * (sc.skin_J | 1) * sizeof(float) : 0);
     auto kern = sc.sh_rows > 0 ? project_bwd_kernel<true> : project_bwd_kernel<false>;
     cudaFuncSetAttribute(kern, cudaFuncAttributeMaxDynamicSharedMemorySize, 128 * 1024);
-    launch_k(kern, (sc.P + 255) / 256, 256, smem, st, true, sc, cx, a, gacc);
+    launch_k(kern, grid, 256, smem, st, true, sc, cx, a, gacc);
   }
   return check_launch();
 }
diff --git a/exavatar_release_b200/plan.py b/exavatar_release_b200/plan.py
--- a/exavatar_release_b200/plan.py
+++ b/exavatar_release_b200/plan.py
@@ -12,7 +12,8 @@
 
 class _Workspace:
 
-    def __init__(self, P: int, width: int, height: int, dup_capacity: int, device, checkpoints: bool = True):
+    def __init__(self, P: int, width: int, height: int, dup_capacity: int, device, checkpoints: bool = True,
+                 split: bool = False):
         self.lib = L.load()
         self.P, self.W, self.H = int(P), int(width), int(height)
         self.device = dev = torch.device(device)
@@ -21,7 +22,8 @@
         self.ctx_bytes = self.lib.b2r_ctx_bytes(P, width, height)
         self.ctx_buf = torch.empty(self.ctx_bytes, dtype=torch.uint8, device=dev)
         self.ids = torch.empty(max(self.capacity, 1), dtype=torch.int32, device=dev)
-        self.scratch_bytes = self.lib.b2r_scratch_bytes(P, width, height, self.capacity)
+        nbytes = self.lib.b2r_split_scratch_bytes if split else self.lib.b2r_scratch_bytes
+        self.scratch_bytes = nbytes(P, width, height, self.capacity)
         self.scratch = torch.empty(self.scratch_bytes, dtype=torch.uint8, device=dev)
         self.bwd_bytes = self.lib.b2r_backward_scratch_bytes(P)
         self.bwd_scratch = torch.zeros(self.bwd_bytes, dtype=torch.uint8, device=dev)
@@ -244,8 +246,8 @@
 
 class _Pass(_Workspace):
 
-    def __init__(self, P, W, H, cap, n_views, device):
-        super().__init__(P, W, H, cap, device)
+    def __init__(self, P, W, H, cap, n_views, device, split=False):
+        super().__init__(P, W, H, cap, device, split=split)
         dev = self.device
         self.ck = [self.ckpt] + [torch.empty_like(self.ckpt) for _ in range(n_views - 1)]
         f = lambda *s: torch.empty(s, dtype=torch.float32, device=dev)
@@ -278,6 +280,7 @@
     PER = FiveRenderPlan.PER
     VIEWS = {"A": ("scene", "human", "scene_human"), "B": ("human_refined", "scene_human_refined")}
     SKIP = os.environ.get("B2R_SKIP_TILES", "1") != "0"
+    SPLIT = SKIP and os.environ.get("B2R_REFINED_PASS", "split") != "full"
 
     def __init__(self, P_scene: int, P_human: int, width: int, height: int, caps: Optional[Dict[str, int]], device,
                  sh_coeffs: int = 0):
@@ -287,7 +290,8 @@
         self.M = int(sh_coeffs)
         self.device = torch.device(device)
         caps = caps or {"A": 8_000_000, "B": 8_000_000}
-        self.passes = {k: _Pass(self.P, self.W, self.H, caps[k], len(v), self.device) for k, v in self.VIEWS.items()}
+        self.passes = {k: _Pass(self.P, self.W, self.H, caps[k], len(v), self.device, split=(k == "B" and self.SPLIT))
+                       for k, v in self.VIEWS.items()}
         self.pass_streams = {k: torch.cuda.Stream(self.device) for k in self.passes}
         lay = merged_bucket_layout(self.Ps, self.Ph, self.M)
         self.all_flat = torch.zeros(lay["total"][1], dtype=torch.float32, device=device)
@@ -361,7 +365,7 @@
         skip = self.Ps if (self.SKIP and name != "scene") else 0
         return L.B2RView(lo, hi, _ptr(bg), fT.data_ptr(), nc.data_ptr(), ps.ck[v].data_ptr(), ps.ckpt_bytes, skip, 0)
 
-    def _start_pass(self, s, pk, key, settings, src, bg_h) -> None:
+    def _start_pass(self, s, pk, key, settings, src, bg_h, a_binned) -> None:
         ps = self.passes[pk]
         if src is not None:
             for k, buf in ps.cat.items():
@@ -369,9 +373,18 @@
         sc = self._scene_desc((key, pk), ps, settings)
         sc.flags = L.B2R_FLAG_CTX_CLEAN if ps.primed else 0
         ps.primed = True
-        L.check(self.lib.b2r_forward_project(C.byref(sc), C.byref(ps.ws), ps.radii.data_ptr(), s.cuda_stream),
-                "b2r_forward_project")
-        L.check(self.lib.b2r_forward_bin(C.byref(sc), C.byref(ps.ws), s.cuda_stream), "b2r_forward_bin")
+        if pk == "B" and self.SPLIT:
+            L.check(self.lib.b2r_forward_project_split(C.byref(sc), C.byref(ps.ws), self.Ps, ps.radii.data_ptr(),
+                                                       s.cuda_stream), "b2r_forward_project_split")
+            s.wait_event(a_binned)
+            L.check(self.lib.b2r_forward_bin_split(C.byref(sc), C.byref(ps.ws), C.byref(self.passes["A"].ws), self.Ps,
+                                                   ps.radii.data_ptr(), s.cuda_stream), "b2r_forward_bin_split")
+        else:
+            L.check(self.lib.b2r_forward_project(C.byref(sc), C.byref(ps.ws), ps.radii.data_ptr(), s.cuda_stream),
+                    "b2r_forward_project")
+            L.check(self.lib.b2r_forward_bin(C.byref(sc), C.byref(ps.ws), s.cuda_stream), "b2r_forward_bin")
+            if pk == "A":
+                a_binned.record(s)
         views = [self._view(ps, v, n, bg_h if n in ("human", "human_refined") else None)
                  for v, n in enumerate(self.VIEWS[pk])]
         self._current[pk] = (sc, views)
@@ -424,14 +437,14 @@
         probe = probe if (probe is not None and serial) else (lambda label: None)
         cur = torch.cuda.current_stream(self.device)
         bg_h = self._human_bg(settings_human_bg)
-        scene_done = torch.cuda.Event()
+        scene_done, a_binned = torch.cuda.Event(), torch.cuda.Event()
         for pk, names in self.VIEWS.items():
             ps = self.passes[pk]
             st = cur if serial else self.pass_streams[pk]
             if not serial:
                 st.wait_stream(cur)
             with torch.cuda.stream(st):
-                self._start_pass(st, pk, key, settings, human if pk == "A" else refined, bg_h)
+                self._start_pass(st, pk, key, settings, human if pk == "A" else refined, bg_h, a_binned)
                 probe(f"{pk}:bin")
                 for v, n in enumerate(names):
                     vs = st if serial else ps.streams[v]
@@ -454,14 +467,14 @@
     def forward_frame(self, key, settings, settings_human_bg, scene, human, refined, copy_inputs: bool = True) -> None:
         cur = torch.cuda.current_stream(self.device)
         bg_h = self._human_bg(settings_human_bg)
-        scene_done = torch.cuda.Event()
+        scene_done, a_binned = torch.cuda.Event(), torch.cuda.Event()
         for pk, names in self.VIEWS.items():
             ps = self.passes[pk]
             st = self.pass_streams[pk]
             st.wait_stream(cur)
             with torch.cuda.stream(st):
                 src = (human if pk == "A" else refined) if copy_inputs else None
-                self._start_pass(st, pk, key, settings, src, bg_h)
+                self._start_pass(st, pk, key, settings, src, bg_h, a_binned)
                 for v in range(len(names)):
                     vs = ps.streams[v]
                     vs.wait_stream(st)
diff --git a/include/b200raster.h b/include/b200raster.h
--- a/include/b200raster.h
+++ b/include/b200raster.h
@@ -158,6 +158,12 @@
 int b2r_backward_project(const B2RScene* scene, const B2RWorkspace* ws, const B2RBackwardArgs* args, void* bwd_scratch,
                          size_t bwd_scratch_bytes, void* stream);
 
+size_t b2r_split_scratch_bytes(int32_t P, int32_t width, int32_t height, uint64_t dup_capacity);
+int b2r_forward_project_split(const B2RScene* scene, const B2RWorkspace* ws, uint32_t first_row, int32_t* radii,
+                              void* stream);
+int b2r_forward_bin_split(const B2RScene* scene, const B2RWorkspace* ws, const B2RWorkspace* base, uint32_t first_row,
+                          int32_t* radii, void* stream);
+
 int b2r_skin_forward(const B2RSkin* skin, void* stream);
 int b2r_skin_backward(const B2RSkin* skin, const float* const dL_dposed[2], float* const dL_dxyz[2], float* dL_djoint,
                       float* dL_dtrans, void* scratch, size_t scratch_bytes, void* stream);
```

After: 1696 (median of 6 runs). +6.0%, better.
